# WeiZhang1988/YDORBSLAM

Measured on AMD Instinct MI355X. Metric: ORB extract+match Mkeypoints/sec, higher is better.
Workload: dtype u8

## Files before the change

### ydorbslam_amd/csrc/extract_kernels.hip.h

```cpp
#pragma once
#include <hip/hip_runtime.h>
#include <stdint.h>

#include "quadtree_core.h"
#include "quadtree_flat.h"

#pragma clang fp contract(off)

namespace ydorb {

constexpr int kPad = 19;
constexpr int kBorder = 16;
constexpr int kMaxLevels = 8;
constexpr int kTileMax = 72;
#ifndef QT_THREADS
#define QT_THREADS 512
#endif
constexpr int kQtThreads = QT_THREADS;

struct LevelDev {
  int w, h, pitch;
  int padOff;
  int blurOff, blurPitch;
  int cellBegin, nCells;
// ... 954 lines not shown
      const int i = t * NT + tid;
      if (i < n && kp[t] < nOut && mm[t] > 16) nodeBig[kp[t]] = 1;
    }
    static_assert(PER <= ITEMS, "the all-pairs candidates live in the first PER state registers");
#pragma unroll
    for (int t = 0; t < PER; t++) st[t] = (st[t] & 0xFFFF0000u) | (uint32_t)(kp[t] < nOut ? kp[t] : 0x7FFF);
    __syncthreads();
  }

#pragma unroll
  for (int g = 0; g < ITEMS / 4; g++) {
    if (!pairs && 4 * g * NT < n) {
      int key[4], slot[4];
#pragma unroll
      for (int jj = 0; jj < 4; jj++) { key[jj] = (int)(st[4 * g + jj] & 0xFFFu); slot[jj] = qf_off(Pn) + (key[jj] >> (2 * (D - Pn))); }
      for (int d = Pn - 1; d >= 1; d--) {
        const int off = qf_off(d), sh = 2 * (D - d);
#pragma unroll
        for (int jj = 0; jj < 4; jj++) {
          const int sl = off + (key[jj] >> sh);
          if (hist[sl] == 1) slot[jj] = sl;
        }
      }
#pragma unroll
      for (int jj = 0; jj < 4; jj++) st[4 * g + jj] = (st[4 * g + jj] & 0xFFFF0000u) | (uint32_t)slot[jj];
    }
  }
  if (!pairs) {
    const int TQ = ((1 << (2 * Pn)) - 1) / 3;
    const int per = (TQ + NT - 1) / NT;
    constexpr int MAXQ = ((1 << (2 * D)) - 1) / 3 / NT + 1;
    uint2 qv[MAXQ];
    int qslot[MAXQ];
    unsigned flags = 0, cntF = 0;
#pragma unroll
    for (int t = 0; t < MAXQ; t++) {
      qslot[t] = -1; qv[t] = make_uint2(0, 0);
      const int q = tid * per + t;
      if (t < per && q < TQ) {
        int d = Pn, start = 0;
        while (q >= start + (1 << (2 * (d - 1)))) { start += 1 << (2 * (d - 1)); d--; }
        const int pq = q - start;
        const int bq = pq ^ (int)(qt_flat_mask(d) >> 2);
        qslot[t] = qf_off(d) + 4 * bq;
        qv[t] = *reinterpret_cast<const QT_LDS uint2*>(hist + qslot[t]);
        const unsigned c[4] = {qv[t].x & 0xFFFFu, qv[t].x >> 16, qv[t].y & 0xFFFFu, qv[t].y >> 16};
        const unsigned sum = c[0] + c[1] + c[2] + c[3];
#pragma unroll
        for (int e = 0; e < 4; e++) {
          const unsigned cn = c[3 - e];
          const bool fl = sum >= 2 && (d == Pn ? cn >= 1 : cn == 1);
          flags |= (unsigned)fl << (4 * t + e);
          cntF += fl;
        }
      }
    }
    unsigned total;
    unsigned pos = block_scan_excl(cntF, &total);
    if ((int)total != K) { give_up(); return; }
#pragma unroll
    for (int t = 0; t < MAXQ; t++) {
      if (qslot[t] >= 0) {
        const unsigned c[4] = {qv[t].x & 0xFFFFu, qv[t].x >> 16, qv[t].y & 0xFFFFu, qv[t].y >> 16};
        unsigned o[4];
#pragma unroll
        for (int e = 0; e < 4; e++) {
          const unsigned cn = c[3 - e];
          unsigned v = 0x7FFFu;
          if ((flags >> (4 * t + e)) & 1u) {
            if ((int)pos < nOut) {
              v = pos | (cn > 16 ? 0x8000u : 0u);
              if (cn > 16) nodeBig[pos] = 1;
            }
            pos++;
          }
          o[3 - e] = v;
        }
        *reinterpret_cast<QT_LDS uint2*>(hist + qslot[t]) = make_uint2(o[0] | (o[1] << 16), o[2] | (o[3] << 16));
      }
    }
  }
  __syncthreads();

#pragma unroll
  for (int g = 0; g < ITEMS / 4; g++) {
    if (4 * g * NT < n) {
      unsigned pv[4];
#pragma unroll
      for (int jj = 0; jj < 4; jj++) pv[jj] = pairs ? st[4 * g + jj] & 0x7FFFu : hist[st[4 * g + jj] & 0xFFFFu] & 0x7FFFu;
#pragma unroll
      for (int jj = 0; jj < 4; jj++) {
        const int i = (4 * g + jj) * NT + tid;
        const bool ok = i < n && (int)pv[jj] < nOut;
        const unsigned k = ok ? pv[jj] : (unsigned)(quotaMax + 1);
        const uint32_t rs = st[4 * g + jj] & 0xFFFF0000u;
        __hip_atomic_fetch_max(nodeLo + k, ok ? rs | (0xFFFFu - (uint32_t)i) : 0u, __ATOMIC_RELAXED, __HIP_MEMORY_SCOPE_WORKGROUP);
        __hip_atomic_fetch_max(nodeHi + k, ok ? rs | (uint32_t)i : 0u, __ATOMIC_RELAXED, __HIP_MEMORY_SCOPE_WORKGROUP);
        st[4 * g + jj] = rs | (ok ? k : 0xFFFFu);
      }
    }
  }
  __syncthreads();
  for (int k = tid; k < nOut; k += NT) {
    const unsigned iLo = 0xFFFFu - (nodeLo[k] & 0xFFFFu), iHi = nodeHi[k] & 0xFFFFu;
    if (iLo == iHi || !nodeBig[k]) {
      outKp[k] = fetch((int)iLo);
    } else {
      const int s = atomicAdd(&sTieN, 1);
      if (s < kQfMaxTied) { sTieNode[s] = k; nodeBig[k] = (uint8_t)(2 + s); }
    }
  }
  __syncthreads();
  const int nTied = sTieN;
  if (nTied > kQfMaxTied) { give_up(); return; }
  if (nTied > 0) {
    const int slotCap = kQfTieCap / nTied;
    QT_LDS uint32_t* tKey = (QT_LDS uint32_t*)smem;
    QT_LDS uint32_t* tVal = tKey + kQfTieCap;
#pragma unroll
    for (int j = 0; j < ITEMS; j++) {
      if (j * NT < n) {
        const unsigned k = st[j] & 0xFFFFu;
        if (k != 0xFFFFu) {
          const unsigned tb = nodeBig[k];
          if (tb >= 2) {
            const int s = (int)tb - 2, idx = atomicAdd(&sTieCnt[s], 1);
            if (idx < slotCap) { tKey[s * slotCap + idx] = (uint32_t)(j * NT + tid); tVal[s * slotCap + idx] = st[j] >> 16; }
            else sFlag = 1;
          }
        }
      }
    }
    __syncthreads();
    if (sFlag) { give_up(); return; }
    for (int s = 0; s < nTied; s++) {
      const int m = sTieCnt[s];
      constexpr int MAXM = (kQfTieCap + NT - 1) / NT;
      int rk[MAXM];
      uint32_t oi[MAXM], rr[MAXM];
#pragma unroll
      for (int t = 0; t < MAXM; t++) {
        rk[t] = -1; oi[t] = 0; rr[t] = 0;
        const int e = tid + NT * t;
        if (e < m) {
          oi[t] = tKey[s * slotCap + e];
          rr[t] = tVal[s * slotCap + e];
          int r = 0;
          for (int u = 0; u < m; u++) r += tKey[s * slotCap + u] < oi[t];
          rk[t] = r;
        }
      }
      __syncthreads();
#pragma unroll
      for (int t = 0; t < MAXM; t++)
        if (rk[t] >= 0) { tKey[s * slotCap + rk[t]] = (rr[t] << 16) | (uint32_t)rk[t]; tVal[s * slotCap + rk[t]] = oi[t]; }
      __syncthreads();
    }
    if (tid < nTied) {
      const int m = sTieCnt[tid];
      const int best = qt_sort_front(tKey + tid * slotCap, m);
      outKp[sTieNode[tid]] = fetch((int)tVal[tid * slotCap + best]);
    }
  }
  if (tid == 0) { needPass[unit] = 0; lvlCount[unit] = nOut; }
}

__global__ __launch_bounds__(256) void k_blur(const uint8_t* __restrict__ pyr, size_t pyrFrameStride, uint8_t* __restrict__ blur,
                                              size_t blurFrameStride, PlanDev P) {
  constexpr int TW = kBlurTW, TH = kBlurTH, SH = TH + 6, SWW = 18;
  __shared__ uint32_t src[SH * SWW];
  __shared__ __align__(16) uint32_t hb[(SH / 2) * TW];
  int f = blockIdx.y, tileId = blockIdx.x;
  if ((f | 7) < (int)gridDim.y) {
    tileId = (f & 7) * (gridDim.x >> 3) + (blockIdx.x >> 3);
    f = (f & ~7) | (blockIdx.x & 7);
  }
  if (tileId >= P.blurTileBegin[P.nLevels]) return;
  int level = 0;
#pragma unroll
  for (int l = 1; l < kMaxLevels; l++)
    if (l < P.nLevels && tileId >= P.blurTileBegin[l]) level = l;
  tileId -= P.blurTileBegin[level];
  const LevelDev L = P.lv[level];
  const int tilesX = (L.w + TW - 1) / TW;
  const int ty = tileId / tilesX, tx = tileId - ty * tilesX;
  const int x0 = tx * TW, y0 = ty * TH;
  const uint8_t* padded = pyr + (size_t)f * pyrFrameStride + L.padOff;
  {
    const int r0 = threadIdx.x / SWW, wd = threadIdx.x - r0 * SWW;
    const int pcol = x0 + 16 + 4 * wd;
    const bool colOk = pcol < L.pitch;
    if (r0 < 14)
#pragma unroll
      for (int r = r0; r < SH; r += 14) {
        const int prow = min(y0 + r + kPad - 3, L.h + 2 * kPad - 1);
        src[r * SWW + wd] = colOk ? *reinterpret_cast<const uint32_t*>(padded + (size_t)prow * L.pitch + pcol) : 0u;
      }
  }
  __syncthreads();
  for (int task = threadIdx.x; task < (SH / 2) * (TW / 4); task += 256) {
    const int rp = task >> 4, g = task & 15;
    uint32_t o[2][4];
#pragma unroll
    for (int h = 0; h < 2; h++) {
      const int r = 2 * rp + h;
      const uint32_t w0 = src[r * SWW + g], w1 = src[r * SWW + g + 1], w2 = src[r * SWW + g + 2];
#pragma unroll
      for (int k = 0; k < 4; k++) {
        const uint32_t lo4 = k ? __builtin_amdgcn_alignbyte(w1, w0, k) : w0, hi4 = k ? __builtin_amdgcn_alignbyte(w2, w1, k) : w1;
        o[h][k] = __builtin_amdgcn_udot4(hi4, 0x00122230u, __builtin_amdgcn_udot4(lo4, 0x38302212u, 0u, false), false);
      }
    }
    *reinterpret_cast<uint4*>(&hb[rp * TW + g * 4]) =
        make_uint4(o[0][0] | (o[1][0] << 16), o[0][1] | (o[1][1] << 16), o[0][2] | (o[1][2] << 16), o[0][3] | (o[1][3] << 16));
  }
  __syncthreads();
  const int c4 = (threadIdx.x & 15) * 4;
#pragma unroll
  for (int r = threadIdx.x >> 4; r < TH; r += 16) {
    const int gy = y0 + r;
    if (!(gy < L.h && x0 + c4 < L.blurPitch)) continue;
    typedef unsigned short u16x2 __attribute__((ext_vector_type(2)));
    const bool odd = r & 1;
    const u16x2 k0 = odd ? u16x2{0, 18} : u16x2{18, 34}, k1 = odd ? u16x2{34, 48} : u16x2{48, 56};
    const u16x2 k2 = odd ? u16x2{56, 48} : u16x2{48, 34}, k3 = odd ? u16x2{34, 18} : u16x2{18, 0};
    const uint32_t* hp = &hb[(r >> 1) * TW + c4];
    const uint4 p0 = *reinterpret_cast<const uint4*>(hp), p1 = *reinterpret_cast<const uint4*>(hp + TW);
    const uint4 p2 = *reinterpret_cast<const uint4*>(hp + 2 * TW), p3 = *reinterpret_cast<const uint4*>(hp + 3 * TW);
    const uint32_t q0[4] = {p0.x, p0.y, p0.z, p0.w}, q1[4] = {p1.x, p1.y, p1.z, p1.w}, q2[4] = {p2.x, p2.y, p2.z, p2.w}, q3[4] = {p3.x, p3.y, p3.z, p3.w};
    uint32_t acc[4];
#pragma unroll
    for (int k = 0; k < 4; k++) {
      acc[k] = __builtin_amdgcn_udot2(__builtin_bit_cast(u16x2, q0[k]), k0, 32768u, false);
      acc[k] = __builtin_amdgcn_udot2(__builtin_bit_cast(u16x2, q1[k]), k1, acc[k], false);
      acc[k] = __builtin_amdgcn_udot2(__builtin_bit_cast(u16x2, q2[k]), k2, acc[k], false);
      acc[k] = __builtin_amdgcn_udot2(__builtin_bit_cast(u16x2, q3[k]), k3, acc[k], false);
    }
    const uint32_t out = (acc[0] >> 16) | ((acc[1] >> 16) << 8) | ((acc[2] >> 16) << 16) | ((acc[3] >> 16) << 24);
    *reinterpret_cast<uint32_t*>(blur + (size_t)f * blurFrameStride + L.blurOff + (size_t)gy * L.blurPitch + x0 + c4) = out;
  }
}

__device__ __forceinline__ float fast_atan2_deg(float y, float x) {
  const float p1 = 0.9997878412794807f * (float)(180 / 3.14159265358979323846);
  const float p3 = -0.3258083974640975f * (float)(180 / 3.14159265358979323846);
  const float p5 = 0.1555786518463281f * (float)(180 / 3.14159265358979323846);
  const float p7 = -0.04432655554792128f * (float)(180 / 3.14159265358979323846);
  const float eps = (float)2.2204460492503131e-16;
  const float ax = fabsf(x), ay = fabsf(y);
  float a, c, c2;
  if (ax >= ay) {
    c = __fdiv_rn(ay, __fadd_rn(ax, eps));
    c2 = __fmul_rn(c, c);
    a = __fmul_rn(__fadd_rn(__fmul_rn(__fadd_rn(__fmul_rn(__fadd_rn(__fmul_rn(p7, c2), p5), c2), p3), c2), p1), c);
  } else {
    c = __fdiv_rn(ax, __fadd_rn(ay, eps));
    c2 = __fmul_rn(c, c);
    a = __fsub_rn(90.f, __fmul_rn(__fadd_rn(__fmul_rn(__fadd_rn(__fmul_rn(__fadd_rn(__fmul_rn(p7, c2), p5), c2), p3), c2), p1), c));
  }
  if (x < 0) a = __fsub_rn(180.f, a);
  if (y < 0) a = __fsub_rn(360.f, a);
  return a;
}

__device__ __forceinline__ void sincos_det(float xf, float* sinOut, float* cosOut) {
  const double x = (double)xf;
  const double n = rint(__dmul_rn(x, 6.36619772367581382433e-01));
  const double r = __dsub_rn(__dsub_rn(x, __dmul_rn(n, 1.57079632673412561417e+00)), __dmul_rn(n, 6.07710050650619224932e-11));
  const double z = __dmul_rn(r, r);
  double p = __dmul_rn(z, 1.58969099521155010221e-10);
  p = __dadd_rn(p, -2.50507602534068634195e-08); p = __dmul_rn(p, z);
  p = __dadd_rn(p, 2.75573137070700676789e-06);  p = __dmul_rn(p, z);
  p = __dadd_rn(p, -1.98412698298579493134e-04); p = __dmul_rn(p, z);
  p = __dadd_rn(p, 8.33333333332248946124e-03);  p = __dmul_rn(p, z);
  p = __dadd_rn(p, -1.66666666666666324348e-01); p = __dmul_rn(p, z);
  p = __dmul_rn(p, r); p = __dadd_rn(p, r);
  double q = __dmul_rn(z, -1.13596475577881948265e-11);
  q = __dadd_rn(q, 2.08757232129817482790e-09);  q = __dmul_rn(q, z);
  q = __dadd_rn(q, -2.75573143513906633035e-07); q = __dmul_rn(q, z);
  q = __dadd_rn(q, 2.48015872894767294178e-05);  q = __dmul_rn(q, z);
  q = __dadd_rn(q, -1.38888888888741095749e-03); q = __dmul_rn(q, z);
  q = __dadd_rn(q, 4.16666666666666019037e-02);  q = __dmul_rn(q, z);
  q = __dmul_rn(q, z);
  double h = __dmul_rn(z, 0.5);
  h = __dsub_rn(h, q);
  h = __dsub_rn(1.0, h);
  const int quad = ((int)n) & 3;
  const double sv = quad == 0 ? p : quad == 1 ? h : quad == 2 ? -p : -h;
  const double cv = quad == 0 ? h : quad == 1 ? -p : quad == 2 ? -h : p;
  *sinOut = (float)sv;
  *cosOut = (float)cv;
}

__device__ __align__(16) const float kPatternDev[1024] = {
#include "orb_pattern_data.inc"
};

struct YdKeyPointDev { float x, y, size, angle, response; int octave, class_id; };

__global__ __launch_bounds__(256) void k_orient_describe(const uint8_t* __restrict__ pyr, size_t pyrFrameStride,
                                                         const uint8_t* __restrict__ blur, size_t blurFrameStride, PlanDev P,
                                                         const uint32_t* __restrict__ lvlKp, const int* __restrict__ lvlCount,
                                                         YdKeyPointDev* __restrict__ kps, uint8_t* __restrict__ desc, int cap,
                                                         int* __restrict__ nOut, float* __restrict__ lvlAngle) {
  const int lane = threadIdx.x & 63;
  int bx = blockIdx.x, f = blockIdx.y;
  if ((f | 7) < (int)gridDim.y) {
    bx = (f & 7) * (gridDim.x >> 3) + (blockIdx.x >> 3);
    f = (f & ~7) | (blockIdx.x & 7);
  }
  const int slot = bx * 4 + __builtin_amdgcn_readfirstlane(threadIdx.x >> 6);
  if (slot >= P.sumQuota) return;
  float4 pat[4];
#pragma unroll
  for (int t = 0; t < 4; t++) pat[t] = reinterpret_cast<const float4*>(kPatternDev)[t * 64 + lane];
  int level = 0;
#pragma unroll
  for (int l = 1; l < kMaxLevels; l++)
    if (l < P.nLevels && slot >= P.lv[l].kpOff) level = l;
  const uint32_t pk = __builtin_amdgcn_readfirstlane(lvlKp[(size_t)f * P.sumQuota + slot]);
  int before = 0, tot = 0, mine = 0;
#pragma unroll
  for (int l = 0; l < kMaxLevels; l++) {
    const int c = l < P.nLevels ? lvlCount[f * kMaxLevels + l] : 0;
    if (l < level) before += c;
    if (l == level) mine = c;
    tot += c;
  }
  if (slot == 0 && lane == 0) nOut[f] = min(tot, cap);
  const LevelDev L = P.lv[level];
  const int k = slot - L.kpOff;
  if (k >= mine) return;
  const int outIdx = before + k;
  if (outIdx >= cap) return;
  const int kx = qt_x(pk) + kBorder, ky = qt_y(pk) + kBorder;
  const uint8_t* roi = pyr + (size_t)f * pyrFrameStride + L.padOff + (size_t)kPad * L.pitch + kPad;
  const uint8_t* org = roi + (ptrdiff_t)(ky - 15) * L.pitch + (kx - 32);
  const int u = lane - 32;
  unsigned narrow = 0;
#pragma unroll
  for (int v = 1; v <= 15; v++) narrow |= (unsigned)(P.maxX[v] == 0) << v;
  int m10 = 0, m01 = 0;
  if (u >= -15 && u <= 15) m10 = u * org[(unsigned)(15 * L.pitch + lane)];
  if (lane >= 1 && lane <= 15 && ((narrow >> lane) & 1u)) {
    const int pos = org[(unsigned)((15 + lane) * L.pitch + 32)], neg = org[(unsigned)((15 - lane) * L.pitch + 32)];
    m01 = lane * (pos - neg);
  }
#pragma unroll
  for (int v = 1; v <= 15; v++) {
    const int d = P.maxX[v];
    if (d > 0 && u >= -d && u <= d) {
      const int pos = org[(unsigned)((15 + v) * L.pitch + lane)], neg = org[(unsigned)((15 - v) * L.pitch + lane)];
      m01 += v * (pos - neg);
      m10 += u * (pos + neg);
    }
  }
#pragma unroll
  for (int o = 32; o >= 1; o >>= 1) {
    m10 += __shfl_xor(m10, o, 64);
    m01 += __shfl_xor(m01, o, 64);
  }
  const float angle = fast_atan2_deg((float)m01, (float)m10);
  const float rad = __fmul_rn(angle, (float)(3.14159265358979323846 / 180.0));
  float sinB, cosA;
  sincos_det(rad, &sinB, &cosA);
  constexpr int kBias = 24;
  const uint8_t* bl = blur + (size_t)f * blurFrameStride + L.blurOff + (ptrdiff_t)(ky - kBias) * L.blurPitch + (kx - kBias);
  unsigned long long words[4];
#pragma unroll
  for (int t = 0; t < 4; t++) {
    const float4 pt = pat[t];
    const int r0 = __float2int_rn(__fadd_rn(__fmul_rn(pt.x, sinB), __fmul_rn(pt.y, cosA)));
    const int c0 = __float2int_rn(__fsub_rn(__fmul_rn(pt.x, cosA), __fmul_rn(pt.y, sinB)));
    const int r1 = __float2int_rn(__fadd_rn(__fmul_rn(pt.z, sinB), __fmul_rn(pt.w, cosA)));
    const int c1 = __float2int_rn(__fsub_rn(__fmul_rn(pt.z, cosA), __fmul_rn(pt.w, sinB)));
    const int t0 = bl[(unsigned)((r0 + kBias) * L.blurPitch + c0 + kBias)], t1 = bl[(unsigned)((r1 + kBias) * L.blurPitch + c1 + kBias)];
    words[t] = __ballot(t0 < t1);
  }
  if (lane < 4) {
    unsigned long long w = lane == 0 ? words[0] : lane == 1 ? words[1] : lane == 2 ? words[2] : words[3];
    reinterpret_cast<unsigned long long*>(desc + ((size_t)f * cap + outIdx) * 32)[lane] = w;
  }
  if (lane == 0) {
    YdKeyPointDev kp;
    kp.x = (float)kx;
    kp.y = (float)ky;
    if (level) { kp.x = __fmul_rn(kp.x, L.scale); kp.y = __fmul_rn(kp.y, L.scale); }
    kp.size = L.size;
    kp.angle = angle;
    kp.response = (float)qt_r(pk);
    kp.octave = level;
    kp.class_id = -1;
    kps[(size_t)f * cap + outIdx] = kp;
    lvlAngle[(size_t)f * P.sumQuota + slot] = angle;
  }
}


template <int KPW>
__global__ __launch_bounds__(256) void k_orient_describe_n(const uint8_t* __restrict__ pyr, size_t pyrFrameStride,
                                                           const uint8_t* __restrict__ blur, size_t blurFrameStride, PlanDev P,
                                                           const uint32_t* __restrict__ lvlKp, const int* __restrict__ lvlCount,
                                                           YdKeyPointDev* __restrict__ kps, uint8_t* __restrict__ desc, int cap,
                                                           int* __restrict__ nOut, float* __restrict__ lvlAngle) {
  const int lane = threadIdx.x & 63;
  int bx = blockIdx.x, f = blockIdx.y;
  if ((f | 7) < (int)gridDim.y) {
    bx = (f & 7) * (gridDim.x >> 3) + (blockIdx.x >> 3);
    f = (f & ~7) | (blockIdx.x & 7);
  }
  const int slot0 = (bx * 4 + __builtin_amdgcn_readfirstlane(threadIdx.x >> 6)) * KPW;
  if (slot0 >= P.sumQuota) return;
  float4 pat[4];
#pragma unroll
  for (int t = 0; t < 4; t++) pat[t] = reinterpret_cast<const float4*>(kPatternDev)[t * 64 + lane];
  int cnt[kMaxLevels], tot = 0;
#pragma unroll
  for (int l = 0; l < kMaxLevels; l++) { cnt[l] = l < P.nLevels ? lvlCount[f * kMaxLevels + l] : 0; tot += cnt[l]; }
  int level[KPW], outIdx[KPW];
  uint32_t pk[KPW];
  bool valid[KPW];
#pragma unroll
  for (int j = 0; j < KPW; j++) {
    const int slot = min(slot0 + j, P.sumQuota - 1);
    level[j] = 0;
#pragma unroll
    for (int l = 1; l < kMaxLevels; l++)
      if (l < P.nLevels && slot >= P.lv[l].kpOff) level[j] = l;
    pk[j] = __builtin_amdgcn_readfirstlane(lvlKp[(size_t)f * P.sumQuota + slot]);
  }
  if (slot0 == 0 && lane == 0) nOut[f] = min(tot, cap);
  bool any = false;
#pragma unroll
  for (int j = 0; j < KPW; j++) {
    int before = 0, mine = 0;
#pragma unroll
    for (int l = 0; l < kMaxLevels; l++) {
      if (l < level[j]) before += cnt[l];
      if (l == level[j]) mine = cnt[l];
    }
    const int k = slot0 + j - P.lv[level[j]].kpOff;
    outIdx[j] = before + k;
    valid[j] = slot0 + j < P.sumQuota && k < mine && outIdx[j] < cap;
    any = any || valid[j];
  }
  if (!any) return;
  int firstValid = 0;
#pragma unroll
  for (int j = KPW - 1; j >= 0; j--) if (valid[j]) firstValid = j;
#pragma unroll
  for (int j = 0; j < KPW; j++)
    if (!valid[j]) {
#pragma unroll
      for (int i = 0; i < KPW; i++) if (i == firstValid) { pk[j] = pk[i]; level[j] = level[i]; }
    }
  int kx[KPW], ky[KPW], pitch[KPW];
  const uint8_t* org[KPW];
#pragma unroll
  for (int j = 0; j < KPW; j++) {
    const LevelDev& L = P.lv[level[j]];
    kx[j] = qt_x(pk[j]) + kBorder; ky[j] = qt_y(pk[j]) + kBorder;
    pitch[j] = L.pitch;
    const uint8_t* roi = pyr + (size_t)f * pyrFrameStride + L.padOff + (size_t)kPad * L.pitch + kPad;
    org[j] = roi + (ptrdiff_t)(ky[j] - 15) * L.pitch + (kx[j] - 32);
  }
  const int u = lane - 32;
  unsigned narrow = 0;
#pragma unroll
  for (int v = 1; v <= 15; v++) narrow |= (unsigned)(P.maxX[v] == 0) << v;
  int m10[KPW], m01[KPW];
#pragma unroll
  for (int j = 0; j < KPW; j++) {
    m10[j] = 0; m01[j] = 0;
    if (u >= -15 && u <= 15) m10[j] = u * org[j][(unsigned)(15 * pitch[j] + lane)];
    if (lane >= 1 && lane <= 15 && ((narrow >> lane) & 1u)) {
      const int pos = org[j][(unsigned)((15 + lane) * pitch[j] + 32)], neg = org[j][(unsigned)((15 - lane) * pitch[j] + 32)];
      m01[j] = lane * (pos - neg);
    }
  }
#pragma unroll
  for (int v = 1; v <= 15; v++) {
    const int d = P.maxX[v];
    if (d > 0 && u >= -d && u <= d) {
#pragma unroll
      for (int j = 0; j < KPW; j++) {
        const int pos = org[j][(unsigned)((15 + v) * pitch[j] + lane)], neg = org[j][(unsigned)((15 - v) * pitch[j] + lane)];
        m01[j] += v * (pos - neg);
        m10[j] += u * (pos + neg);
      }
    }
  }
#pragma unroll
  for (int o = 32; o >= 1; o >>= 1) {
#pragma unroll
    for (int j = 0; j < KPW; j++) {
      m10[j] += __shfl_xor(m10[j], o, 64);
      m01[j] += __shfl_xor(m01[j], o, 64);
    }
  }
  constexpr int kBias = 24;
  float angle[KPW];
  int tA[KPW][4], tB[KPW][4];
#pragma unroll
  for (int j = 0; j < KPW; j++) {
    const LevelDev& L = P.lv[level[j]];
    angle[j] = fast_atan2_deg((float)m01[j], (float)m10[j]);
    const float rad = __fmul_rn(angle[j], (float)(3.14159265358979323846 / 180.0));
    float sinB, cosA;
    sincos_det(rad, &sinB, &cosA);
    const uint8_t* bl = blur + (size_t)f * blurFrameStride + L.blurOff + (ptrdiff_t)(ky[j] - kBias) * L.blurPitch + (kx[j] - kBias);
#pragma unroll
    for (int t = 0; t < 4; t++) {
      const float4 pt = pat[t];
      const int r0 = __float2int_rn(__fadd_rn(__fmul_rn(pt.x, sinB), __fmul_rn(pt.y, cosA)));
      const int c0 = __float2int_rn(__fsub_rn(__fmul_rn(pt.x, cosA), __fmul_rn(pt.y, sinB)));
      const int r1 = __float2int_rn(__fadd_rn(__fmul_rn(pt.z, sinB), __fmul_rn(pt.w, cosA)));
      const int c1 = __float2int_rn(__fsub_rn(__fmul_rn(pt.z, cosA), __fmul_rn(pt.w, sinB)));
      tA[j][t] = bl[(unsigned)((r0 + kBias) * L.blurPitch + c0 + kBias)];
      tB[j][t] = bl[(unsigned)((r1 + kBias) * L.blurPitch + c1 + kBias)];
    }
  }
#pragma unroll
  for (int j = 0; j < KPW; j++) {
    unsigned long long words[4];
#pragma unroll
    for (int t = 0; t < 4; t++) words[t] = __ballot(tA[j][t] < tB[j][t]);
    if (!valid[j]) continue;
    const LevelDev& L = P.lv[level[j]];
    if (lane < 4) {
      unsigned long long w = lane == 0 ? words[0] : lane == 1 ? words[1] : lane == 2 ? words[2] : words[3];
      reinterpret_cast<unsigned long long*>(desc + ((size_t)f * cap + outIdx[j]) * 32)[lane] = w;
    }
    if (lane == 0) {
      YdKeyPointDev kp;
      kp.x = (float)kx[j];
      kp.y = (float)ky[j];
      if (level[j]) { kp.x = __fmul_rn(kp.x, L.scale); kp.y = __fmul_rn(kp.y, L.scale); }
      kp.size = L.size;
      kp.angle = angle[j];
      kp.response = (float)qt_r(pk[j]);
      kp.octave = level[j];
      kp.class_id = -1;
      kps[(size_t)f * cap + outIdx[j]] = kp;
      lvlAngle[(size_t)f * P.sumQuota + slot0 + j] = angle[j];
    }
  }
}

}
```

### ydorbslam_amd/csrc/orb_extractor.hip

```cpp
#include <hip/hip_runtime.h>
#include <cstdlib>

#include <algorithm>
#include <cmath>
#include <cstdarg>
#include <cstdio>
#include <cstring>
#include <string>
#include <vector>

#include "../../include/ydorb/c_api.h"
#include "extract_kernels.hip.h"
#include "host_buffers.h"
#include "ydorb_host.h"

using namespace ydorb;

namespace {

inline int cvRoundF(float v) { return (int)lrintf(v); }
inline int cvFloorF(float v) { int i = (int)v; return i - (i > v); }
inline int alignUp(int v, int a) { return (v + a - 1) / a * a; }
inline size_t alignUpZ(size_t v, size_t a) { return (v + a - 1) / a * a; }

struct HostPlan {
  int w = 0, h = 0;
  PlanDev dev{};
  std::vector<CellDev> cells;
  size_t pyrFrameStride = 0, blurFrameStride = 0, qtFrameStride = 0;
  int maxCellDim = 0;
  int levelCellDim[kMaxLevels]{};
  struct QtLevel { int nodeCap, candCap; size_t lds; int items; bool passOk; } qt[kMaxLevels]{};
  size_t qtLdsMax = 0;
  size_t qtPassLds = 0;
  int qtPassNodes = 0;
  std::vector<int> tabInt;
  std::vector<short> tabShort;
  struct TabOff { int xofs, yofs, alpha, beta; } tab[kMaxLevels]{};
  struct FusedLevel { bool on = false; int shift = 0, padOff = 0, colOff = 0, rowOff = 0; } fused[kMaxLevels];
  std::vector<PyrPadEntry> padTab;
  std::vector<PyrColEntry> colTab;
  std::vector<int2> rowTab;
};

enum Stage { ST_PYR = 0, ST_FAST, ST_QT, ST_BLUR, ST_DESC, ST_COUNT };
const char* kStageNames[ST_COUNT] = {"pyramid", "fast_cells", "blur", "quadtree_after_blur", "orient_describe"};

struct TablePtrs { CellDev* cells; int* tabInt; short* tabShort; PyrPadEntry* padTab; PyrColEntry* colTab; int2* rowTab; };
size_t layTables(const HostPlan& P, void* base, TablePtrs& t) {
  Carve a(base);
  a.take(t.cells, P.cells.size()); a.take(t.tabInt, P.tabInt.size()); a.take(t.tabShort, P.tabShort.size());
  a.take(t.padTab, P.padTab.size()); a.take(t.colTab, P.colTab.size()); a.take(t.rowTab, P.rowTab.size());
  return a.L.bytes;
}

struct WorkPtrs {
  uint8_t *pyr, *blur; uint32_t *cellCount, *cellCand, *qtCand; uint16_t* qtNode; uint8_t* nodeScratch; uint32_t* lvlKp; float* lvlAngle; int* lvlCount;
  uint8_t* needPass; int *lvlMaxN, *status, *passList;
};
size_t layWork(const HostPlan& P, size_t B, void* base, WorkPtrs& w) {
  const PlanDev& D = P.dev;
  Carve a(base);
  a.take(w.pyr, P.pyrFrameStride * B); a.take(w.blur, P.blurFrameStride * B);
  a.take(w.cellCount, D.nCellsTotal * B); a.take(w.cellCand, (size_t)D.nCellsTotal * D.cellCap * B);
  a.take(w.qtCand, 2 * P.qtFrameStride * B); a.take(w.qtNode, 2 * P.qtFrameStride * B); a.take(w.nodeScratch, D.nodeTabFrameStride * B);
  a.take(w.lvlKp, D.sumQuota * B); a.take(w.lvlAngle, D.sumQuota * B); a.take(w.lvlCount, kMaxLevels * B);
  a.take(w.needPass, kMaxLevels * B); a.take(w.lvlMaxN, kMaxLevels + 1); a.take(w.status, 1); a.take(w.passList, kMaxLevels * B + 1);
  return a.L.bytes;
}

struct IoPtrs { uint8_t* img; YdKeyPoint* kps; uint8_t* desc; int* nOut; };
size_t layIo(size_t imgBytes, size_t Q, size_t B, void* base, IoPtrs& p) {
  static_assert(sizeof(YdKeyPoint) == sizeof(YdKeyPointDev), "one layout for the device and the pinned staging");
  Carve a(base);
  a.take(p.img, imgBytes * B); a.take(p.kps, Q * B); a.take(p.desc, 32 * Q * B); a.take(p.nOut, B);
  return a.L.bytes;
}

}

struct ydorb_extractor {
  YdExtractorConfig cfg{};
  std::vector<float> sf, isf, sf2, isf2;
  std::vector<int> perLevel;
  int maxX[16]{};
  int sumQuota = 0;
  hipStream_t stream = nullptr;
  hipStream_t qtStream[kMaxLevels]{};
  hipEvent_t evFork = nullptr, evJoin[kMaxLevels]{};
  hipEvent_t evFast[kMaxLevels]{};
  int descKpw = 2;
  bool qtInline = false;
  int fastGroups = 1;
  HostPlan plan;
  bool planValid = false;
  int batchCap = 0;
  size_t imgBytes = 0;
  Mem tables;
  Mem work;
  Mem io; PinnedMem hIo;
  PinnedMem hSync;
  PinnedMem h_pyr;
  TablePtrs tab{};
  WorkPtrs d{};
  IoPtrs dIo{}, hIoAt{};
  int *h_lvlMaxN = nullptr, *h_status = nullptr;
  std::vector<Mem*> buffers() { return {&tables, &work, &io, &hIo, &hSync, &h_pyr}; }
  hipStream_t lastStream = nullptr;
  int lastFrames = 0;
  bool noFusedPads = false;
  bool profiling = false;
  bool profPending = false;
  bool forcePassQuadtree = false;
  hipEvent_t ev[ST_COUNT + 1]{};
  double stageMs[ST_COUNT]{};
  int stageCalls = 0;
};

namespace {

void release(ydorb_extractor* e) {
  for (Mem* b : e->buffers()) b->release();
  e->planValid = false;
  e->lastStream = nullptr; e->lastFrames = 0;
}

int syncStreams(ydorb_extractor* e) {
  HIPCHK(hipStreamSynchronize(e->stream));
  if (e->lastStream && e->lastStream != e->stream) HIPCHK(hipStreamSynchronize(e->lastStream));
  return YDORB_OK;
}


static int qfItemsFor(long want) { return want <= 8L * kQfThreads ? 8 : want <= 16L * kQfThreads ? 16 : 32; }

void buildFusedLevel(HostPlan& P, int l) {
  const PlanDev& D = P.dev;
  const LevelDev& L = D.lv[l];
  HostPlan::FusedLevel& F = P.fused[l];
  F.on = false;
  if (L.w < 20 || L.h < 20) return;
  const int nd = (L.w + 2 * kPad + 3) >> 2;
  auto srcOf = [&](int p) { return p < kPad ? 2 * kPad - p : p < kPad + L.w ? -1 : p < L.w + 2 * kPad ? 2 * L.w + 2 * kPad - 2 - p : -2; };
  int shift = -1;
  for (int sft = 0; sft < 64 && shift < 0; sft++) {
    bool ok = true;
    for (int c = 0; c < nd && ok; c++)
      for (int j = 0; j < 4; j++) {
        const int sp = srcOf(4 * c + j);
        if (sp >= 0 && ((sp >> 2) + sft) >> 6 != (c + sft) >> 6) ok = false;
      }
    if (ok) shift = sft;
  }
  if (shift < 0) return;
  std::vector<PyrColEntry> col;
  if (l > 0) {
    const LevelDev& Lp = D.lv[l - 1];
    const int* xofs = P.tabInt.data() + P.tab[l].xofs;
    const short* alpha = P.tabShort.data() + P.tab[l].alpha;
    col.resize(nd);
    for (int c = 0; c < nd; c++) {
      const int dx0 = std::min(std::max(4 * c - kPad, 0), L.w - 1);
      for (int b = 0; b < 4; b++) {
        const int dx = std::min(std::max(4 * c - kPad + b, 0), L.w - 1);
        const int off = xofs[dx] - xofs[dx0];
        if (off < 0 || off > 6 || xofs[dx0] + 7 >= Lp.w + kPad) return;
        col[c].sel[b] = (uint32_t)off | 0x0c000c00u | ((uint32_t)(off + 1) << 16);
        col[c].ab[b] = (uint32_t)(uint16_t)alpha[2 * dx] | ((uint32_t)(uint16_t)alpha[2 * dx + 1] << 16);
      }
    }
  }
  F.shift = shift;
  F.padOff = (int)P.padTab.size();
  for (int c = 0; c < nd; c++) {
    int dA = -1, dB = -1;
    for (int j = 0; j < 4; j++) {
      const int sp = srcOf(4 * c + j);
      if (sp < 0) continue;
      const int d = sp >> 2;
      if (dA < 0 || d == dA) dA = d;
      else dB = d;
    }
    PyrPadEntry pe{};
    pe.laneA4 = 4u * (unsigned)(((dA < 0 ? c : dA) + shift) & 63);
    pe.laneB4 = 4u * (unsigned)(((dB < 0 ? c : dB) + shift) & 63);
    pe.selM = 0; pe.selF = 0;
    for (int j = 0; j < 4; j++) {
      const int sp = srcOf(4 * c + j);
      uint32_t m = 0x0c, f;
      if (sp == -1) f = (uint32_t)j;
      else if (sp == -2) f = 0x0c;
      else { m = (uint32_t)(sp & 3) + ((sp >> 2) == dA ? 4u : 0u); f = 4u + (uint32_t)j; }
      pe.selM |= m << (8 * j);
      pe.selF |= f << (8 * j);
    }
    P.padTab.push_back(pe);
  }
  if (l > 0) {
    F.colOff = (int)P.colTab.size();
    P.colTab.insert(P.colTab.end(), col.begin(), col.end());
    F.rowOff = (int)P.rowTab.size();
    const int* yofs = P.tabInt.data() + P.tab[l].yofs;
    const short* beta = P.tabShort.data() + P.tab[l].beta;
    const int rows = alignUp(L.h, 4 * kPyrRowsF);
    for (int y = 0; y < rows; y++) {
      const int dy = std::min(y, L.h - 1);
      P.rowTab.push_back(make_int2(yofs[dy], (int)((uint32_t)(uint16_t)beta[2 * dy] | ((uint32_t)(uint16_t)beta[2 * dy + 1] << 16))));
    }
  }
  F.on = true;
}

int buildPlan(ydorb_extractor* e, int w, int h, HostPlan& P) {
  P = HostPlan();
  P.w = w; P.h = h;
  PlanDev& D = P.dev;
  D.nLevels = e->cfg.n_levels;
  for (int v = 0; v < 16; v++) D.maxX[v] = e->maxX[v];
  size_t padOff = 0, blurOff = 0;
  int kpOff = 0, candOff = 0, maxCellDim = 0;
  for (int l = 0; l < D.nLevels; l++) {
    LevelDev& L = D.lv[l];
    L.w = cvRoundF((float)w * e->isf[l]);
    L.h = cvRoundF((float)h * e->isf[l]);
    if (L.w < 1 || L.h < 1 || L.w > 4000 || L.h > 4000) {
      set_error("level %d size %dx%d out of the supported range (1..4000)", l, L.w, L.h);
      return YDORB_ERR_UNSUPPORTED;
    }
    L.pitch = alignUp(L.w + 2 * kPad, 64);
    L.padOff = (int)padOff;
    padOff += alignUpZ((size_t)(L.h + 2 * kPad) * L.pitch, 256);
    L.blurPitch = alignUp(L.w, 64);
    L.blurOff = (int)blurOff;
    blurOff += alignUpZ((size_t)L.h * L.blurPitch, 256);
    L.quota = e->perLevel[l];
    L.kpOff = kpOff;
    kpOff += L.quota;
    L.scale = e->sf[l];
    L.size = (float)(int)(31 * e->sf[l]);
    L.cellBegin = (int)P.cells.size();
    const int minB = kBorder, maxBX = L.w - kBorder, maxBY = L.h - kBorder;
    const float width = (float)(maxBX - minB), height = (float)(maxBY - minB);
    const int colsNum = (int)(width / 30.0f), rowsNum = (int)(height / 30.0f);
    if (colsNum > 0 && rowsNum > 0) {
      const int cellW = (int)ceilf(width / colsNum), cellH = (int)ceilf(height / rowsNum);
      maxCellDim = std::max(maxCellDim, std::max(cellW, cellH));
      P.levelCellDim[l] = std::max(cellW, cellH);
      for (int i = 0; i < rowsNum; i++) {
        const float iniY = (float)(minB + i * cellH);
        float maxY = iniY + cellH + 6;
        if (iniY >= maxBY - 3) continue;
        if (maxY > maxBY) maxY = (float)maxBY;
        for (int j = 0; j < colsNum; j++) {
          const float iniX = (float)(minB + j * cellW);
          float maxX = iniX + cellW + 6;
          if (iniX >= maxBX - 6) continue;
          if (maxX > maxBX) maxX = (float)maxBX;
          CellDev c{};
          c.level = (short)l;
          c.x0 = (short)iniX; c.y0 = (short)iniY; c.x1 = (short)maxX; c.y1 = (short)maxY;
          c.srcOff = L.padOff + (kPad + c.y0) * L.pitch + kPad + c.x0;
          P.cells.push_back(c);
        }
      }
    }
    L.nCells = (int)P.cells.size() - L.cellBegin;
    if (l > 0) {
      const LevelDev& Lp = D.lv[l - 1];
      const double scale_x = 1. / ((double)L.w / Lp.w), scale_y = 1. / ((double)L.h / Lp.h);
      P.tab[l].xofs = (int)P.tabInt.size();
      P.tab[l].alpha = (int)P.tabShort.size();
      for (int dx = 0; dx < L.w; dx++) {
        float fx = (float)((dx + 0.5) * scale_x - 0.5);
        int sx = cvFloorF(fx);
        fx -= sx;
        if (sx < 0) { fx = 0; sx = 0; }
        if (sx >= Lp.w - 1) { fx = 0; sx = Lp.w - 1; }
        P.tabInt.push_back(sx);
        P.tabShort.push_back((short)cvRoundF((1.f - fx) * 2048));
        P.tabShort.push_back((short)cvRoundF(fx * 2048));
      }
      P.tab[l].yofs = (int)P.tabInt.size();
      P.tab[l].beta = (int)P.tabShort.size();
      for (int dy = 0; dy < L.h; dy++) {
        float fy = (float)((dy + 0.5) * scale_y - 0.5);
        int sy = cvFloorF(fy);
        fy -= sy;
        P.tabInt.push_back(sy);
        P.tabShort.push_back((short)cvRoundF((1.f - fy) * 2048));
        P.tabShort.push_back((short)cvRoundF(fy * 2048));
      }
    }
  }
  if (maxCellDim + 6 > kTileMax) {
    set_error("cell size %d exceeds the FAST tile (%d)", maxCellDim, kTileMax - 6);
    return YDORB_ERR_UNSUPPORTED;
  }
  D.nCellsTotal = (int)P.cells.size();
  P.maxCellDim = maxCellDim;
  D.cellCap = alignUp(std::max(((maxCellDim + 1) / 2) * ((maxCellDim + 1) / 2), 64), 64);
  D.sumQuota = kpOff;
  for (int l = 0; l < D.nLevels; l++) {
    D.lv[l].candOff = candOff;
    candOff += D.lv[l].nCells * D.cellCap;
  }
  for (int l = 0; l < D.nLevels && !e->noFusedPads; l++) buildFusedLevel(P, l);
  D.borderBegin[0] = 0;
  for (int l = 0; l < kMaxLevels; l++)
    D.borderBegin[l + 1] = D.borderBegin[l] + (l < D.nLevels && !P.fused[l].on ? alignUp(2 * kPad * (D.lv[l].pitch / 4) + 12 * D.lv[l].h, 256) : 0);
  D.blurTileBegin[0] = 0;
  for (int l = 0; l < kMaxLevels; l++)
    D.blurTileBegin[l + 1] = D.blurTileBegin[l] + (l < D.nLevels ? ((D.lv[l].w + kBlurTW - 1) / kBlurTW) * ((D.lv[l].h + kBlurTH - 1) / kBlurTH) : 0);
  P.pyrFrameStride = padOff;
  P.blurFrameStride = blurOff;
  P.qtFrameStride = (size_t)candOff;
  for (int l = 0; l < D.nLevels; l++) {
    const LevelDev& L = D.lv[l];
    HostPlan::QtLevel& Q = P.qt[l];
    Q.nodeCap = 4 * std::max(L.quota, 1);
    const long band = (long)std::max(L.w - 2 * kBorder, 1) * std::max(L.h - 2 * kBorder, 1);
    Q.candCap = (int)std::min<long>(4608, std::max<long>(512, band / 22)) / 64 * 64;
    Q.lds = (size_t)Q.nodeCap * 48 + (size_t)Q.candCap * 12 + (size_t)(L.nCells + 1) * 4;
    if (Q.lds > 150 * 1024) {
      Q.candCap = 0;
      Q.lds = (size_t)Q.nodeCap * 48 + (size_t)(L.nCells + 1) * 4;
    }
    Q.passOk = Q.lds <= 150 * 1024;
    if (Q.passOk) {
      P.qtLdsMax = std::max(P.qtLdsMax, Q.lds);
      P.qtPassLds = std::max(P.qtPassLds, (size_t)Q.nodeCap * 48 + (size_t)(L.nCells + 1) * 4);
      P.qtPassNodes = std::max(P.qtPassNodes, Q.nodeCap);
      D.lv[l].nodeTabOff = -1;
    } else {
      if (Q.nodeCap > 65535) { set_error("n_features=%d: level %d would need %d quad-tree nodes (max 65535)", e->cfg.n_features, l, Q.nodeCap); return YDORB_ERR_UNSUPPORTED; }
      D.lv[l].nodeTabOff = (int)D.nodeTabFrameStride;
      D.nodeTabFrameStride += (unsigned)alignUpZ((size_t)Q.nodeCap * 48, 256);
      Q.candCap = 0;
      Q.lds = (size_t)(L.nCells + 1) * 4 + 64;
      P.qtLdsMax = std::max(P.qtLdsMax, Q.lds);
      P.qtPassLds = std::max(P.qtPassLds, Q.lds);
    }
    Q.items = qfItemsFor((long)((double)band / (45.0 - 3.5 * l)) + 64);
  }
  P.qtPassLds = std::max<size_t>(P.qtPassLds, 1024);
  return YDORB_OK;
}

size_t fastGeom(const HostPlan& P, int la, int lb, FastLds& fl, bool& narrow) {
  int dim = 1;
  for (int l = la; l < lb; l++) dim = std::max(dim, P.levelCellDim[l]);
  const int maxT = dim + 6, maxB = dim;
  narrow = maxT <= 44;
  const int pitch = narrow ? 48 : 80;
  fl.tileBytes = alignUp((maxT + 3) * pitch, 16);
  fl.scoreBytes = alignUp((maxB + 2) * (maxB + 2) + 4, 16);
  fl.listBytes = alignUp(2 * maxB * maxB, 16);
  return (size_t)4 * (fl.tileBytes + fl.scoreBytes + fl.listBytes);
}

template <class T> void copyTable(T* dst, const std::vector<T>& v) { if (!v.empty()) memcpy(dst, v.data(), sizeof(T) * v.size()); }

int ensurePlan(ydorb_extractor* e, int w, int h, int nFrames) {
  if (e->planValid && e->plan.w == w && e->plan.h == h && nFrames <= e->batchCap) return YDORB_OK;
  int rc = syncStreams(e);
  if (rc) return rc;
  HostPlan P;
  if ((rc = buildPlan(e, w, h, P))) return rc;
  release(e);
  const size_t B = std::max(nFrames, std::max(1, e->cfg.max_batch));
  const PlanDev& D = P.dev;
  std::vector<uint8_t> hTables(layTables(P, nullptr, e->tab));
  if ((rc = e->tables.alloc(hTables.size())) || (rc = e->work.alloc(layWork(P, B, nullptr, e->d))) ||
      (rc = e->hSync.alloc(sizeof(int) * (kMaxLevels + 2)))) return rc;
  layWork(P, B, e->work.p, e->d);
  e->h_lvlMaxN = e->hSync.as<int>();
  e->h_status = e->h_lvlMaxN + kMaxLevels + 1;
  memset(e->hSync.p, 0, e->hSync.cap);
  TablePtrs ht;
  layTables(P, hTables.data(), ht);
  copyTable(ht.cells, P.cells); copyTable(ht.tabInt, P.tabInt); copyTable(ht.tabShort, P.tabShort);
  copyTable(ht.padTab, P.padTab); copyTable(ht.colTab, P.colTab); copyTable(ht.rowTab, P.rowTab);
  layTables(P, e->tables.p, e->tab);
  if (!hTables.empty()) HIPCHK(hipMemcpyAsync(e->tables.p, hTables.data(), hTables.size(), hipMemcpyHostToDevice, e->stream));
  HIPCHK(hipMemsetAsync(e->d.pyr, 0, P.pyrFrameStride * B, e->stream));
  HIPCHK(hipMemsetAsync(e->d.needPass, 0, (uint8_t*)(e->d.passList + 1) - e->d.needPass, e->stream));
  HIPCHK(hipStreamSynchronize(e->stream));
  e->plan = P;
  e->batchCap = (int)B;
  e->imgBytes = (size_t)w * h;
  {
    FastLds fl; bool narrow;
    const size_t dynAll = fastGeom(P, 0, D.nLevels, fl, narrow);
    if (dynAll > 48 * 1024) {
      HIPCHK(hipFuncSetAttribute(reinterpret_cast<const void*>(k_fast_cells<48>), hipFuncAttributeMaxDynamicSharedMemorySize, (int)dynAll));
      HIPCHK(hipFuncSetAttribute(reinterpret_cast<const void*>(k_fast_cells<80>), hipFuncAttributeMaxDynamicSharedMemorySize, (int)dynAll));
    }
  }
  if (std::max(P.qtLdsMax, P.qtPassLds) > 48 * 1024)
  {
    HIPCHK(hipFuncSetAttribute(reinterpret_cast<const void*>(k_quadtree), hipFuncAttributeMaxDynamicSharedMemorySize, (int)std::max(P.qtLdsMax, P.qtPassLds)));
    HIPCHK(hipFuncSetAttribute(reinterpret_cast<const void*>(k_quadtree_list), hipFuncAttributeMaxDynamicSharedMemorySize, (int)std::max(P.qtLdsMax, P.qtPassLds)));
  }
  {
    int qmax = 1, tabLen = 2;
    for (int l = 0; l < D.nLevels; l++) { qmax = std::max(qmax, D.lv[l].quota); tabLen = std::max(tabLen, std::max(D.lv[l].w - 2 * kBorder, 0) + std::max(D.lv[l].h - 2 * kBorder, 0) + 2); }
    const size_t ldsFast = std::min<size_t>(qt_fast_lds_bytes(qmax, tabLen), 150 * 1024);
    if (ldsFast > 48 * 1024) {
      HIPCHK(hipFuncSetAttribute(reinterpret_cast<const void*>(k_qt_fast<8>), hipFuncAttributeMaxDynamicSharedMemorySize, (int)ldsFast));
      HIPCHK(hipFuncSetAttribute(reinterpret_cast<const void*>(k_qt_fast<16>), hipFuncAttributeMaxDynamicSharedMemorySize, (int)ldsFast));
      HIPCHK(hipFuncSetAttribute(reinterpret_cast<const void*>(k_qt_fast<32>), hipFuncAttributeMaxDynamicSharedMemorySize, (int)ldsFast));
    }
  }
  e->planValid = true;
  return YDORB_OK;
}

int ensureIo(ydorb_extractor* e) {
  if (e->io.p && e->hIo.p) return YDORB_OK;
  const size_t bytes = layIo(e->imgBytes, e->sumQuota, e->batchCap, nullptr, e->dIo);
  int rc;
  if ((rc = e->io.alloc(bytes)) || (rc = e->hIo.alloc(bytes))) return rc;
  layIo(e->imgBytes, e->sumQuota, e->batchCap, e->io.p, e->dIo);
  layIo(e->imgBytes, e->sumQuota, e->batchCap, e->hIo.p, e->hIoAt);
  return YDORB_OK;
}

void collectProfile(ydorb_extractor* e);

static void retuneQuadtree(ydorb_extractor* e) {
  HostPlan& P = e->plan;
  for (int l = 0; l < P.dev.nLevels; l++) {
    const int seen = e->h_lvlMaxN[l];
    if (seen > 0) P.qt[l].items = qfItemsFor((long)seen + seen / 8 + 32);
  }
}

int enqueue(ydorb_extractor* e, const uint8_t* d_img, int stride, size_t frameStride, int nFrames, YdKeyPointDev* d_kps,
            uint8_t* d_desc, int cap, int* d_nOut, hipStream_t s) {
  retuneQuadtree(e);
  const HostPlan& P = e->plan;
  const PlanDev& D = P.dev;
  const bool prof = e->profiling;
  if (prof) {
    if (e->profPending && hipEventQuery(e->ev[ST_COUNT]) == hipSuccess) collectProfile(e);
    e->profPending = false;
    HIPCHK(hipEventRecord(e->ev[0], s));
  }
  {
    const LevelDev& L0 = D.lv[0];
    auto fusedGrid = [&](const LevelDev& L, int shift) {
      return dim3((((L.w + 2 * kPad + 3) >> 2) + shift + 63) / 64, (L.h + 4 * kPyrRowsF - 1) / (4 * kPyrRowsF), nFrames);
    };
    if (P.fused[0].on) {
      hipLaunchKernelGGL(k_pyr_level0_f, fusedGrid(L0, P.fused[0].shift), dim3(256), 0, s, d_img, stride, frameStride, e->d.pyr, P.pyrFrameStride, L0,
                         e->tab.padTab + P.fused[0].padOff, P.fused[0].shift);
    } else {
      dim3 g((L0.pitch / 4 + 63) / 64, (L0.h + 4 * kPyrRows - 1) / (4 * kPyrRows), nFrames);
      hipLaunchKernelGGL(k_pyr_level0, g, dim3(256), 0, s, d_img, stride, frameStride, e->d.pyr, P.pyrFrameStride, L0);
    }
    for (int l = 1; l < D.nLevels; l++) {
      const LevelDev& L = D.lv[l];
      const double scaleX = 1. / ((double)L.w / D.lv[l - 1].w);
      if (P.fused[l].on) {
        const HostPlan::FusedLevel& F = P.fused[l];
        hipLaunchKernelGGL(k_pyr_resize_f, fusedGrid(L, F.shift), dim3(256), 0, s, e->d.pyr, P.pyrFrameStride, D.lv[l - 1], L, scaleX,
                           e->tab.colTab + F.colOff, e->tab.padTab + F.padOff, e->tab.rowTab + F.rowOff, F.shift);
      } else {
        dim3 gl((L.pitch / 4 + 63) / 64, (L.h + 4 * kPyrRows - 1) / (4 * kPyrRows), nFrames);
        hipLaunchKernelGGL(k_pyr_resize, gl, dim3(256), 0, s, e->d.pyr, P.pyrFrameStride, D.lv[l - 1], L, scaleX,
                           e->tab.tabShort + P.tab[l].alpha, e->tab.tabInt + P.tab[l].yofs, e->tab.tabShort + P.tab[l].beta);
      }
    }
    if (D.borderBegin[D.nLevels] > 0)
      hipLaunchKernelGGL(k_pyr_borders, dim3(D.borderBegin[D.nLevels] / 256, nFrames), dim3(256), 0, s, e->d.pyr, P.pyrFrameStride, D);
  }
  if (prof) HIPCHK(hipEventRecord(e->ev[1], s));
  hipEvent_t fastEv[kMaxLevels]{};
  int grpFirst[kMaxLevels]{}, grpEnd[kMaxLevels]{}, nGroups = 0;
  {
    const int thr = std::min(std::max(e->cfg.ini_fast_thr, 0), 255);
    int l0 = 0;
    for (int g = 0; g < e->fastGroups && l0 < D.nLevels; g++) {
      const int l1 = g == e->fastGroups - 1 ? D.nLevels : l0 + 1;
      const int c0 = D.lv[l0].cellBegin, c1 = D.lv[l1 - 1].cellBegin + D.lv[l1 - 1].nCells;
      if (c1 > c0 && D.nCellsTotal > 0) {
        FastLds fl; bool narrow;
        const size_t dyn = fastGeom(P, l0, l1, fl, narrow);
        const dim3 grid(((c1 - c0 + 3) / 4 + 7) / 8 * 8, nFrames);
        if (narrow) hipLaunchKernelGGL(k_fast_cells<48>, grid, dim3(256), dyn, s, e->d.pyr, P.pyrFrameStride, D, e->tab.cells, c0, c1, thr, fl, e->d.cellCount, e->d.cellCand);
        else hipLaunchKernelGGL(k_fast_cells<80>, grid, dim3(256), dyn, s, e->d.pyr, P.pyrFrameStride, D, e->tab.cells, c0, c1, thr, fl, e->d.cellCount, e->d.cellCand);
      }
      HIPCHK(hipEventRecord(e->evFast[l0], s));
      fastEv[l0] = e->evFast[l0];
      grpFirst[nGroups] = l0; grpEnd[nGroups] = l1; nGroups++;
      for (int l = l0 + 1; l < l1; l++) fastEv[l] = e->evFast[l0];
      l0 = l1;
    }
  }
  if (prof) HIPCHK(hipEventRecord(e->ev[2], s));
  HIPCHK(hipEventRecord(e->evFork, s));
  hipLaunchKernelGGL(k_blur, dim3((D.blurTileBegin[D.nLevels] + 7) / 8 * 8, nFrames), dim3(256), 0, s, e->d.pyr, P.pyrFrameStride, e->d.blur,
                     P.blurFrameStride, D);
  if (prof) HIPCHK(hipEventRecord(e->ev[3], s));
  bool anyFast = false;
  for (int g = 0; g < nGroups; g++) {
    const int l0 = grpFirst[g], l1 = grpEnd[g];
    const hipStream_t qs = e->qtInline ? s : e->qtStream[g % kMaxLevels];
    if (!e->qtInline) HIPCHK(hipStreamWaitEvent(qs, fastEv[l0] ? fastEv[l0] : e->evFork, 0));
    int items = 8, qmax = 1, tabLen = 2;
    for (int l = l0; l < l1; l++) {
      items = std::max(items, P.qt[l].items); qmax = std::max(qmax, D.lv[l].quota);
      tabLen = std::max(tabLen, std::max(D.lv[l].w - 2 * kBorder, 0) + std::max(D.lv[l].h - 2 * kBorder, 0) + 2);
    }
    const size_t lds = qt_fast_lds_bytes(qmax, tabLen);
    if (!e->forcePassQuadtree && lds <= 150 * 1024) {
      const dim3 grid(nFrames, l1 - l0);
#define YD_QT_FAST(IT) hipLaunchKernelGGL(k_qt_fast<IT>, grid, dim3(kQfThreads), lds, qs, D, e->d.cellCount, e->d.cellCand, l0, qmax, tabLen, e->d.lvlKp, \
                                          e->d.lvlCount, e->d.needPass, e->d.lvlMaxN, e->d.passList, e->d.passList + 1)
      if (items <= 8) YD_QT_FAST(8);
      else if (items <= 16) YD_QT_FAST(16);
      else YD_QT_FAST(32);
#undef YD_QT_FAST
      anyFast = true;
    } else {
      for (int l = l0; l < l1; l++) {
        const HostPlan::QtLevel& Q = P.qt[l];
        hipLaunchKernelGGL(k_quadtree, dim3(1, nFrames), dim3(kQtThreads), Q.lds, qs, D, e->d.cellCount, e->d.cellCand, e->d.qtCand, e->d.qtNode,
                           P.qtFrameStride, Q.nodeCap, Q.candCap, l, e->d.lvlKp, e->d.lvlCount, e->d.status, e->d.nodeScratch);
      }
    }
    if (!e->qtInline) HIPCHK(hipEventRecord(e->evJoin[g], qs));
  }
  if (!e->qtInline) for (int g = 0; g < nGroups; g++) HIPCHK(hipStreamWaitEvent(s, e->evJoin[g], 0));
  if (anyFast) {
    const int seen = e->h_lvlMaxN[kMaxLevels];
    const int listGrid = std::max(1, std::min({kQtPassWorkgroups, D.nLevels * nFrames, seen + seen / 4}));
    hipLaunchKernelGGL(k_quadtree_list, dim3(listGrid), dim3(kQtListThreads), P.qtPassLds, s, D, e->d.cellCount, e->d.cellCand,
                       e->d.qtCand, e->d.qtNode, P.qtFrameStride, -std::max(P.qtPassNodes, 1), e->d.lvlKp, e->d.lvlCount, e->d.status, e->d.passList,
                       e->d.passList + 1, e->d.nodeScratch, e->d.lvlMaxN + kMaxLevels);
    HIPCHK(hipMemsetAsync(e->d.passList, 0, sizeof(int), s));
  }
  if (prof) HIPCHK(hipEventRecord(e->ev[4], s));
  {
    const int kpw = e->descKpw;
    const dim3 gd(((D.sumQuota + 4 * kpw - 1) / (4 * kpw) + 7) / 8 * 8, nFrames);
#define YD_DESC(K) hipLaunchKernelGGL((k_orient_describe_n<K>), gd, dim3(256), 0, s, e->d.pyr, P.pyrFrameStride, e->d.blur, P.blurFrameStride, D, \
                                         e->d.lvlKp, e->d.lvlCount, d_kps, d_desc, cap, d_nOut, e->d.lvlAngle)
    if (kpw == 1)
      hipLaunchKernelGGL(k_orient_describe, gd, dim3(256), 0, s, e->d.pyr, P.pyrFrameStride, e->d.blur,
                         P.blurFrameStride, D, e->d.lvlKp, e->d.lvlCount, d_kps, d_desc, cap, d_nOut, e->d.lvlAngle);
    else if (kpw == 2) YD_DESC(2);
    else YD_DESC(4);
#undef YD_DESC
  }
  if (prof) { HIPCHK(hipEventRecord(e->ev[5], s)); e->profPending = true; }
  HIPCHK(hipMemcpyAsync(e->h_lvlMaxN, e->d.lvlMaxN, sizeof(int) * (kMaxLevels + 1), hipMemcpyDeviceToHost, s));
  HIPCHK(hipGetLastError());
  e->lastFrames = nFrames;
  e->lastStream = s;
  return YDORB_OK;
}

int checkStatus(ydorb_extractor* e) {
  if (*e->h_status == 1) { set_error("more than 65535 FAST candidates in one pyramid level"); return YDORB_ERR_CAPACITY; }
  if (*e->h_status == 3) { set_error("a pyramid level needs the pass quad-tree kernel (more candidates than LDS slots, or a very deep tree) but its quota is too large for that kernel's LDS node table"); return YDORB_ERR_CAPACITY; }
  if (*e->h_status) { set_error("quad-tree node table overflow (status %d)", *e->h_status); return YDORB_ERR_CAPACITY; }
  return YDORB_OK;
}

void collectProfile(ydorb_extractor* e) {
  if (!e->profiling || !e->profPending) return;
  e->profPending = false;
  for (int i = 0; i < ST_COUNT; i++) {
    float ms = 0;
    if (hipEventElapsedTime(&ms, e->ev[i], e->ev[i + 1]) == hipSuccess) e->stageMs[i] += ms;
  }
  e->stageCalls++;
}

}

int ydorb::extractor_pyramid_view(const ydorb_extractor* e, PyramidView* v) {
  if (!e || !v || !e->planValid || e->lastFrames < 1) { set_error("the extractor holds no pyramid (no call yet)"); return YDORB_ERR_INVALID_ARG; }
  v->device = e->cfg.device; v->nLevels = e->cfg.n_levels; v->frames = e->lastFrames; v->frameStride = (long long)e->plan.pyrFrameStride;
  v->stream = e->stream;
  for (int l = 0; l < e->cfg.n_levels; l++) {
    const LevelDev& L = e->plan.dev.lv[l];
    v->roi[l] = e->d.pyr + L.padOff + (size_t)kPad * L.pitch + kPad;
    v->w[l] = L.w; v->h[l] = L.h; v->pitch[l] = L.pitch;
    v->scale[l] = e->sf[l]; v->invScale[l] = e->isf[l];
    v->quota[l] = e->perLevel[l];
  }
  return YDORB_OK;
}

extern "C" {

int ydorb_extractor_create(const YdExtractorConfig* cfg, ydorb_extractor_t** out) {
  if (!cfg || !out) { set_error("null argument"); return YDORB_ERR_INVALID_ARG; }
  *out = nullptr;
  if (cfg->n_levels < 1 || cfg->n_levels > kMaxLevels || cfg->n_features < 1 || !(cfg->scale_factor > 1.0f)) {
    set_error("unsupported extractor config (n_levels 1..8, n_features >= 1, scale_factor > 1)");
    return YDORB_ERR_INVALID_ARG;
  }
  int rc = ydorb::require_device(cfg->device);
  if (rc) return rc;
  ydorb_extractor* e = new ydorb_extractor();
  e->cfg = *cfg;
  if (const char* v = getenv("YDORB_QT_PASS")) e->forcePassQuadtree = v[0] == '1';
  if (const char* v = getenv("YDORB_PYR_FUSED")) e->noFusedPads = v[0] == '0';
  e->descKpw = cfg->max_batch <= 8 ? 1 : 4;
  if (const char* v = getenv("YDORB_DESC_KPW")) e->descKpw = atoi(v) == 1 ? 1 : atoi(v) == 4 ? 4 : 2;
  e->cfg.min_fast_thr = cfg->ini_fast_thr;
  const int L = cfg->n_levels;
  const float s = cfg->scale_factor;
  int per = (int)round(cfg->n_features * (1 - 1.0 / s) / (1.0 - pow(1.0 / s, L)));
  int sum = 0;
  for (int i = 0; i < L; i++) {
    e->sf.push_back((float)pow(s, i));
    e->sf2.push_back((float)pow(s, 2 * i));
    e->isf.push_back((float)pow(s, -i));
    e->isf2.push_back((float)pow(s, -2 * i));
    if (i < L - 1) {
      e->perLevel.push_back(per);
      sum += per;
      per = (int)round((float)per / s);
    } else {
      e->perLevel.push_back(std::max(cfg->n_features - sum, 0));
    }
  }
  e->sumQuota = 0;
  for (int q : e->perLevel) e->sumQuota += q;
  {
    const int half = 15;
    std::vector<int> mx(half + 1, 0);
    const int maxY = (int)floor(half * sqrt(2.0) / 2.0 + 1.0), minY = (int)ceil(half * sqrt(2.0) / 2.0);
    for (int v = 0; v <= maxY; v++) mx.push_back((int)round(sqrt((double)half * half + (double)v * v)));
    for (int v = half, i = 0; v >= minY; v--) {
      while (mx[i] == mx[i + 1]) i++;
      mx[v] = i;
      i++;
    }
    for (int v = 0; v < 16; v++) e->maxX[v] = mx[v];
  }
  if (hipStreamCreateWithFlags(&e->stream, hipStreamNonBlocking) != hipSuccess) {
    set_error("hipStreamCreate failed");
    delete e;
    return YDORB_ERR_HIP;
  }
  for (auto& ev : e->ev) (void)hipEventCreate(&ev);
  (void)hipEventCreateWithFlags(&e->evFork, hipEventDisableTiming);
  for (int l = 0; l < kMaxLevels; l++) {
    const char* qtEnv = getenv("YDORB_QT_STREAMS");
    e->qtInline = (qtEnv && atoi(qtEnv) == 0) || (cfg->flags & YDORB_EXTRACTOR_SINGLE_STREAM);
    const int nQt = std::max(1, std::min(qtEnv ? atoi(qtEnv) : (cfg->max_batch <= 8 ? (int)kMaxLevels : 2), (int)kMaxLevels));
    if (l < nQt) (void)hipStreamCreateWithFlags(&e->qtStream[l], hipStreamNonBlocking);
    else e->qtStream[l] = e->qtStream[l % nQt];
    (void)hipEventCreateWithFlags(&e->evJoin[l], hipEventDisableTiming);
    (void)hipEventCreateWithFlags(&e->evFast[l], hipEventDisableTiming);
  }
  {
    const char* g = getenv("YDORB_FAST_GROUPS");
    e->fastGroups = std::max(1, std::min(g ? atoi(g) : (cfg->max_batch <= 8 ? 1 : 2), (int)kMaxLevels));
  }
  *out = e;
  return YDORB_OK;
}

void ydorb_extractor_destroy(ydorb_extractor_t* e) {
  if (!e) return;
  (void)hipSetDevice(e->cfg.device);
  if (e->stream) (void)hipStreamSynchronize(e->stream);
  release(e);
  for (auto& ev : e->ev) if (ev) (void)hipEventDestroy(ev);
  for (int l = 0; l < kMaxLevels; l++) {
    if (e->qtStream[l]) {
      bool shared = false;
      for (int k = 0; k < l; k++) shared = shared || e->qtStream[k] == e->qtStream[l];
      if (!shared) { (void)hipStreamSynchronize(e->qtStream[l]); (void)hipStreamDestroy(e->qtStream[l]); }
    }
    if (e->evJoin[l]) (void)hipEventDestroy(e->evJoin[l]);
    if (e->evFast[l]) (void)hipEventDestroy(e->evFast[l]);
  }
  if (e->evFork) (void)hipEventDestroy(e->evFork);
  if (e->stream) (void)hipStreamDestroy(e->stream);
  delete e;
}

int ydorb_extractor_tables(const ydorb_extractor_t* e, float* scale, float* inv_scale, float* scale_sq, float* inv_scale_sq,
                           int32_t* per_level) {
  if (!e) { set_error("null handle"); return YDORB_ERR_INVALID_ARG; }
  for (int i = 0; i < e->cfg.n_levels; i++) {
    if (scale) scale[i] = e->sf[i];
    if (inv_scale) inv_scale[i] = e->isf[i];
    if (scale_sq) scale_sq[i] = e->sf2[i];
    if (inv_scale_sq) inv_scale_sq[i] = e->isf2[i];
    if (per_level) per_level[i] = e->perLevel[i];
  }
  return YDORB_OK;
}

int ydorb_extractor_max_keypoints(const ydorb_extractor_t* e) { return e ? e->sumQuota : YDORB_ERR_INVALID_ARG; }

int ydorb_extract_batch_device(ydorb_extractor_t* e, const uint8_t* d_img, int32_t w, int32_t h, int32_t stride, size_t frame_stride,
                               int32_t n_frames, YdKeyPoint* d_kps, uint8_t* d_desc, int32_t cap, int32_t* d_n_out, void* stream) {
  if (!e || !d_img || !d_kps || !d_desc || !d_n_out || w <= 0 || h <= 0 || n_frames <= 0 || stride < w) {
    set_error("invalid argument");
    return YDORB_ERR_INVALID_ARG;
  }
  if (cap < e->sumQuota) { set_error("cap %d < max keypoints %d", cap, e->sumQuota); return YDORB_ERR_CAPACITY; }
  HIPCHK(hipSetDevice(e->cfg.device));
  int rc = ensurePlan(e, w, h, n_frames);
  if (rc) return rc;
  return enqueue(e, d_img, stride, frame_stride, n_frames, reinterpret_cast<YdKeyPointDev*>(d_kps), d_desc, cap, d_n_out,
                 stream ? (hipStream_t)stream : e->stream);
}

int ydorb_extractor_synchronize(ydorb_extractor_t* e) {
  if (!e) { set_error("null handle"); return YDORB_ERR_INVALID_ARG; }
  HIPCHK(hipSetDevice(e->cfg.device));
  int rc = syncStreams(e);
  if (rc || !e->planValid) return rc;
  HIPCHK(hipMemcpy(e->h_status, e->d.status, sizeof(int), hipMemcpyDeviceToHost));
  rc = checkStatus(e);
  if (rc) HIPCHK(hipMemset(e->d.status, 0, sizeof(int)));
  return rc;
}

int ydorb_extract_batch(ydorb_extractor_t* e, const uint8_t* img, int32_t w, int32_t h, int32_t stride, size_t frame_stride,
                        int32_t n_frames, YdKeyPoint* kps, uint8_t* desc, int32_t cap, int32_t* n_out) {
  if (!e || !n_out) { set_error("null argument"); return YDORB_ERR_INVALID_ARG; }
  if (!img || w <= 0 || h <= 0 || n_frames <= 0) {
    for (int f = 0; f < std::max(n_frames, 0); f++) n_out[f] = 0;
    return YDORB_OK;
  }
  if (!kps || !desc || stride < w) { set_error("invalid argument"); return YDORB_ERR_INVALID_ARG; }
  HIPCHK(hipSetDevice(e->cfg.device));
  int rc = ensurePlan(e, w, h, n_frames);
  if (rc || (rc = ensureIo(e))) return rc;
  const int Q = e->sumQuota;
  YdKeyPointDev* d_kps = reinterpret_cast<YdKeyPointDev*>(e->dIo.kps);
  for (int f = 0; f < n_frames; f++)
    for (int y = 0; y < h; y++) memcpy(e->hIoAt.img + (size_t)f * e->imgBytes + (size_t)y * w, img + f * frame_stride + (size_t)y * stride, w);
  HIPCHK(hipMemcpyAsync(e->dIo.img, e->hIoAt.img, e->imgBytes * n_frames, hipMemcpyHostToDevice, e->stream));
  rc = enqueue(e, e->dIo.img, w, e->imgBytes, n_frames, d_kps, e->dIo.desc, Q, e->dIo.nOut, e->stream);
  if (rc) return rc;
  HIPCHK(hipMemcpyAsync(e->hIoAt.nOut, e->dIo.nOut, sizeof(int) * n_frames, hipMemcpyDeviceToHost, e->stream));
  HIPCHK(hipMemcpyAsync(e->h_status, e->d.status, sizeof(int), hipMemcpyDeviceToHost, e->stream));
  HIPCHK(hipMemcpyAsync(e->hIoAt.kps, d_kps, sizeof(YdKeyPoint) * (size_t)Q * n_frames, hipMemcpyDeviceToHost, e->stream));
  HIPCHK(hipMemcpyAsync(e->hIoAt.desc, e->dIo.desc, (size_t)32 * Q * n_frames, hipMemcpyDeviceToHost, e->stream));
  HIPCHK(hipStreamSynchronize(e->stream));
  collectProfile(e);
  rc = checkStatus(e);
  if (rc) {
    HIPCHK(hipMemset(e->d.status, 0, sizeof(int)));
    return rc;
  }
  for (int f = 0; f < n_frames; f++) {
    const int n = e->hIoAt.nOut[f];
    if (n > cap) { set_error("frame %d has %d keypoints, caller capacity %d", f, n, cap); return YDORB_ERR_CAPACITY; }
    memcpy(kps + (size_t)f * cap, e->hIoAt.kps + (size_t)f * Q, sizeof(YdKeyPoint) * n);
    memcpy(desc + (size_t)f * cap * 32, e->hIoAt.desc + (size_t)f * Q * 32, (size_t)32 * n);
    n_out[f] = n;
  }
  return YDORB_OK;
}

int ydorb_extract(ydorb_extractor_t* e, const uint8_t* img, int32_t w, int32_t h, int32_t stride, YdKeyPoint* kps, uint8_t* desc,
                  int32_t cap, int32_t* n_out) {
  return ydorb_extract_batch(e, img, w, h, stride, 0, 1, kps, desc, cap, n_out);
}

int ydorb_extractor_pyramid(const ydorb_extractor_t* e, int32_t frame, int32_t level, const uint8_t** d_roi, int32_t* w, int32_t* h,
                            int32_t* stride) {
  if (!e || !e->planValid || frame < 0 || frame >= e->lastFrames || level < 0 || level >= e->cfg.n_levels) {
    set_error("no pyramid for frame %d level %d", frame, level);
    return YDORB_ERR_INVALID_ARG;
  }
  const LevelDev& L = e->plan.dev.lv[level];
  if (d_roi) *d_roi = e->d.pyr + (size_t)frame * e->plan.pyrFrameStride + L.padOff + (size_t)kPad * L.pitch + kPad;
  if (w) *w = L.w;
  if (h) *h = L.h;
  if (stride) *stride = L.pitch;
  return YDORB_OK;
}

int ydorb_extractor_read_level(ydorb_extractor_t* e, int32_t frame, int32_t level, uint8_t* dst, size_t dst_bytes) {
  const uint8_t* roi;
  int w, h, stride;
  int rc = ydorb_extractor_pyramid(e, frame, level, &roi, &w, &h, &stride);
  if (rc) return rc;
  const size_t need = (size_t)(w + 2 * kPad) * (h + 2 * kPad);
  if (!dst || dst_bytes < need) { set_error("need %zu bytes", need); return YDORB_ERR_CAPACITY; }
  HIPCHK(hipSetDevice(e->cfg.device));
  HIPCHK(hipStreamSynchronize(e->stream));
  HIPCHK(hipMemcpy2D(dst, w + 2 * kPad, roi - (size_t)kPad * stride - kPad, stride, w + 2 * kPad, h + 2 * kPad, hipMemcpyDeviceToHost));
  return YDORB_OK;
}

int ydorb_extractor_read_pyramid(ydorb_extractor_t* e, int32_t frame, uint8_t* const* dst_levels, const size_t* dst_bytes, int32_t n_levels) {
  if (!e || !e->planValid || frame < 0 || frame >= e->lastFrames || !dst_levels || !dst_bytes || n_levels < 1 || n_levels > e->cfg.n_levels) {
    set_error("invalid argument");
    return YDORB_ERR_INVALID_ARG;
  }
  const HostPlan& P = e->plan;
  for (int l = 0; l < n_levels; l++) {
    const LevelDev& L = P.dev.lv[l];
    const size_t need = (size_t)(L.w + 2 * kPad) * (L.h + 2 * kPad);
    if (!dst_levels[l] || dst_bytes[l] < need) { set_error("level %d needs %zu bytes", l, need); return YDORB_ERR_CAPACITY; }
  }
  HIPCHK(hipSetDevice(e->cfg.device));
  if (const int rc = e->h_pyr.ensure(P.pyrFrameStride)) return rc;
  const uint8_t* h_pyr = e->h_pyr.as<uint8_t>();
  hipStream_t s = e->lastStream ? e->lastStream : e->stream;
  HIPCHK(hipMemcpyAsync(e->h_pyr.p, e->d.pyr + (size_t)frame * P.pyrFrameStride, P.pyrFrameStride, hipMemcpyDeviceToHost, s));
  HIPCHK(hipStreamSynchronize(s));
  for (int l = 0; l < n_levels; l++) {
    const LevelDev& L = P.dev.lv[l];
    const int rowBytes = L.w + 2 * kPad;
    for (int y = 0; y < L.h + 2 * kPad; y++) memcpy(dst_levels[l] + (size_t)y * rowBytes, h_pyr + L.padOff + (size_t)y * L.pitch, rowBytes);
  }
  return YDORB_OK;
}

int ydorb_extractor_debug_read(ydorb_extractor_t* e, int32_t what, int32_t frame, int32_t level, void* dst, size_t dst_bytes,
                               size_t* written) {
  if (!e || !e->planValid || frame < 0 || frame >= e->lastFrames || level < 0 || level >= e->cfg.n_levels || !dst || !written) {
    set_error("invalid argument");
    return YDORB_ERR_INVALID_ARG;
  }
  HIPCHK(hipSetDevice(e->cfg.device));
  HIPCHK(hipStreamSynchronize(e->stream));
  const HostPlan& P = e->plan;
  const PlanDev& D = P.dev;
  const LevelDev& L = D.lv[level];
  if (what == 0) {
    const size_t need = (size_t)L.w * L.h;
    if (dst_bytes < need) { set_error("need %zu bytes", need); return YDORB_ERR_CAPACITY; }
    HIPCHK(hipMemcpy2D(dst, L.w, e->d.blur + (size_t)frame * P.blurFrameStride + L.blurOff, L.blurPitch, L.w, L.h, hipMemcpyDeviceToHost));
    *written = need;
    return YDORB_OK;
  }
  if (what == 1) {
    std::vector<uint32_t> cnt(L.nCells), buf((size_t)L.nCells * D.cellCap);
    if (L.nCells) {
      HIPCHK(hipMemcpy(cnt.data(), e->d.cellCount + (size_t)frame * D.nCellsTotal + L.cellBegin, sizeof(uint32_t) * L.nCells, hipMemcpyDeviceToHost));
      HIPCHK(hipMemcpy(buf.data(), e->d.cellCand + ((size_t)frame * D.nCellsTotal + L.cellBegin) * D.cellCap,
                       sizeof(uint32_t) * buf.size(), hipMemcpyDeviceToHost));
    }
    YdKeyPoint* o = (YdKeyPoint*)dst;
    size_t n = 0;
    for (int c = 0; c < L.nCells; c++)
      for (uint32_t i = 0; i < cnt[c]; i++) {
        if ((n + 1) * sizeof(YdKeyPoint) > dst_bytes) { set_error("candidate buffer too small"); return YDORB_ERR_CAPACITY; }
        const uint32_t pk = buf[(size_t)c * D.cellCap + i];
        o[n++] = YdKeyPoint{(float)qt_x(pk), (float)qt_y(pk), 7.f, -1.f, (float)qt_r(pk), 0, -1};
      }
    *written = n * sizeof(YdKeyPoint);
    return YDORB_OK;
  }
  if (what == 2) {
    int counts[kMaxLevels];
    HIPCHK(hipMemcpy(counts, e->d.lvlCount + frame * kMaxLevels, sizeof(counts), hipMemcpyDeviceToHost));
    const int n = counts[level];
    if ((size_t)n * sizeof(YdKeyPoint) > dst_bytes) { set_error("keypoint buffer too small"); return YDORB_ERR_CAPACITY; }
    std::vector<uint32_t> pk(std::max(n, 1));
    std::vector<float> ang(std::max(n, 1));
    if (n) {
      HIPCHK(hipMemcpy(pk.data(), e->d.lvlKp + (size_t)frame * D.sumQuota + L.kpOff, sizeof(uint32_t) * n, hipMemcpyDeviceToHost));
      HIPCHK(hipMemcpy(ang.data(), e->d.lvlAngle + (size_t)frame * D.sumQuota + L.kpOff, sizeof(float) * n, hipMemcpyDeviceToHost));
    }
    YdKeyPoint* o = (YdKeyPoint*)dst;
    for (int i = 0; i < n; i++)
      o[i] = YdKeyPoint{(float)(qt_x(pk[i]) + kBorder), (float)(qt_y(pk[i]) + kBorder), L.size, ang[i], (float)qt_r(pk[i]), level, -1};
    *written = (size_t)n * sizeof(YdKeyPoint);
    return YDORB_OK;
  }
  if (what == 3) {
    if (dst_bytes < 1) { set_error("need 1 byte"); return YDORB_ERR_CAPACITY; }
    uint8_t v = 1;
    int qmaxAll = 1, tabAll = 2;
    for (int l = 0; l < D.nLevels; l++) { qmaxAll = std::max(qmaxAll, D.lv[l].quota); tabAll = std::max(tabAll, std::max(D.lv[l].w - 2 * kBorder, 0) + std::max(D.lv[l].h - 2 * kBorder, 0) + 2); }
    if (!e->forcePassQuadtree && qt_fast_lds_bytes(qmaxAll, tabAll) <= 150 * 1024)
      HIPCHK(hipMemcpy(&v, e->d.needPass + (size_t)frame * kMaxLevels + level, 1, hipMemcpyDeviceToHost));
    *(uint8_t*)dst = v;
    *written = 1;
    return YDORB_OK;
  }
  set_error("unknown debug stage %d", what);
  return YDORB_ERR_INVALID_ARG;
}

int ydorb_extractor_set_profiling(ydorb_extractor_t* e, int32_t on) {
  if (!e) return YDORB_ERR_INVALID_ARG;
  e->profiling = on != 0;
  for (double& m : e->stageMs) m = 0;
  e->stageCalls = 0;
  return YDORB_OK;
}

int ydorb_extractor_stage_times(ydorb_extractor_t* e, int32_t max_stages, const char** names, float* ms, int32_t* n_stages) {
  if (!e || !n_stages) return YDORB_ERR_INVALID_ARG;
  if (e->profiling && e->profPending) {
    if (hipEventSynchronize(e->ev[ST_COUNT]) == hipSuccess) collectProfile(e);
  }
  const int n = std::min<int>(max_stages, ST_COUNT);
  for (int i = 0; i < n; i++) {
    if (names) names[i] = kStageNames[i];
    if (ms) ms[i] = e->stageCalls ? (float)(e->stageMs[i] / e->stageCalls) : 0.f;
  }
  *n_stages = n;
  return YDORB_OK;
}

}
```

### ydorbslam_amd/csrc/orb_matcher.hip

```cpp
#include <hip/hip_runtime.h>

#include <algorithm>
#include <cstdlib>
#include <cmath>
#include <cstring>
#include <vector>

#include "../../include/ydorb/c_api.h"
#include "frustum_kernels.hip.h"
#include "host_buffers.h"
#include "match_kernels.hip.h"
#include "stereo_kernels.hip.h"
#include "ydorb_host.h"

using namespace ydorb;

namespace {

int launchGridBuild(int nFrames, int cap, hipStream_t s, const FrameDev* frames) {
  const size_t dyn = sizeof(int16_t) * (size_t)std::max(cap, 0);
  if (dyn > 48 * 1024)
    HIPCHK(hipFuncSetAttribute(reinterpret_cast<const void*>(k_grid_build), hipFuncAttributeMaxDynamicSharedMemorySize, (int)dyn));
  hipLaunchKernelGGL(k_grid_build, dim3(nFrames), dim3(256), dyn, s, frames, cap);
  HIPCHK(hipGetLastError());
  return YDORB_OK;
}

__global__ void k_hamming_rows(const uint8_t* a, const uint8_t* b, int n, int* out) {
  const int i = blockIdx.x * 256 + threadIdx.x;
  if (i < n) out[i] = hamming256(a + (size_t)i * 32, b + (size_t)i * 32);
}

enum { MS_GRID = 0, MS_GATHER, MS_RESOLVE, MS_COUNT };
const char* kMatchStageNames[MS_COUNT] = {"grid_build", "gather_distances", "resolve"};

constexpr size_t kTakenPad = 31;

template <class Lay> int layOut(Mem& arena, Lay lay) {
  const int rc = arena.ensure(lay(nullptr));
  if (rc == YDORB_OK) lay(arena.p);
  return rc;
}

struct BatchPtrs {
  FrameDev* frames; CallDev* calls; float *sf, *ident;
  QueryDev* queries; uint8_t* taken; int* matchQ; int2* qInfo; uint2* qPre; unsigned* heads;
  int *cellStart, *cellIdx; float4* sortedKp; uint8_t* sortedDesc;
  uint32_t* pool;
};
size_t layBatch(size_t cap, size_t nCalls, size_t nFrames, size_t poolPerCall, void* base, BatchPtrs& p) {
  Carve a(base);
  a.take(p.frames, nFrames); a.take(p.calls, nCalls); a.take(p.sf, 8); a.take(p.ident, 6 * nCalls);
  a.take(p.queries, cap * nCalls); a.take(p.taken, cap * nCalls + kTakenPad); a.take(p.matchQ, cap * nCalls); a.take(p.qInfo, cap * nCalls);
  a.take(p.qPre, cap * nCalls); a.take(p.heads, nCalls); a.take(p.cellStart, (kGridCells + 1) * nFrames); a.take(p.cellIdx, cap * nFrames);
  a.take(p.sortedKp, cap * nFrames); a.take(p.sortedDesc, 32 * cap * nFrames);
  a.take(p.pool, poolPerCall * nCalls);
  return a.L.bytes;
}

struct ProjPtrs {
  int* status; FrameDev* frame; CallDev* call;
  KeyPointDev* kps; uint8_t* desc; float* rightX; int *cellStart, *cellIdx; float4* sortedKp; uint8_t* sortedDesc;
  QueryDev* queries; uint8_t *qdesc, *taken; int *assigned, *matchQ; int2* qInfo; uint2* qPre;
  uint8_t *table, *track;
};
size_t layProjection(size_t n, bool stereo, size_t nq, size_t tableBytes, size_t trackBytes, void* base, ProjPtrs& p) {
  Carve a(base);
  a.take(p.status, 16); a.take(p.frame, 1); a.take(p.call, 1);
  a.take(p.kps, n); a.take(p.desc, 32 * n); a.take(p.rightX, stereo ? n : 0); a.take(p.cellStart, kGridCells + 1); a.take(p.cellIdx, n);
  a.take(p.sortedKp, n); a.take(p.sortedDesc, 32 * n);
  a.take(p.queries, nq); a.take(p.qdesc, 32 * nq); a.take(p.taken, n + kTakenPad); a.take(p.assigned, n); a.take(p.matchQ, nq); a.take(p.qInfo, nq);
  a.take(p.qPre, nq); a.take(p.table, tableBytes); a.take(p.track, trackBytes);
  return a.L.bytes;
}

struct BowPtrs {
  int* status; CallDev* call;
  uint8_t *descA, *descB, *valid, *goodA, *goodB; KeyPointDev *kpsA, *kpsB; int *feat, *qFeat, *assigned, *matchQ; int2 *qRange, *qInfo; float* qAngle;
};
size_t layBow(size_t nA, size_t nB, size_t nFeatB, size_t nq, bool tri, void* base, BowPtrs& p) {
  Carve a(base);
  a.take(p.status, 16); a.take(p.call, 1);
  a.take(p.descA, 32 * nA); a.take(p.descB, 32 * nB); a.take(p.kpsB, nB); a.take(p.feat, nFeatB); a.take(p.valid, nB);
  a.take(p.qFeat, nq); a.take(p.qRange, nq); a.take(p.qAngle, nq); a.take(p.qInfo, nq); a.take(p.matchQ, nq); a.take(p.assigned, std::max(nq, nB));
  a.take(p.kpsA, tri ? nA : 0); a.take(p.goodA, tri ? nA : 0); a.take(p.goodB, tri ? nB : 0);
  return a.L.bytes;
}

struct RowsPtrs { uint8_t *a, *b; int *offsets, *idx, *out; TopkOut* top; };
size_t layRows(size_t nA, size_t nB, size_t nOffsets, size_t nIdx, size_t nOut, size_t nTop, void* base, RowsPtrs& r) {
  Carve a(base);
  a.take(r.a, 32 * nA); a.take(r.b, 32 * nB); a.take(r.offsets, nOffsets); a.take(r.idx, nIdx); a.take(r.out, nOut); a.take(r.top, nTop);
  return a.L.bytes;
}

struct StereoPtrs { int *counters, *kept, *status, *nL, *nR; KeyPointDev *kpsL, *kpsR; uint8_t *descL, *descR; float *rightX, *depth; };
size_t layStereo(size_t nPairs, size_t nl, size_t nr, void* base, StereoPtrs& p) {
  Carve a(base);
  a.take(p.counters, 4 * nPairs); a.take(p.kept, nPairs); a.take(p.status, nPairs);
  a.take(p.kpsL, nl); a.take(p.descL, 32 * nl); a.take(p.kpsR, nr); a.take(p.descR, 32 * nr); a.take(p.nL, nl ? nPairs : 0); a.take(p.nR, nl ? nPairs : 0);
  a.take(p.rightX, nl); a.take(p.depth, nl);
  return a.L.bytes;
}

}

struct ydorb_matcher {
  int device = 0;
  hipStream_t stream = nullptr;
  Mem call;
  Mem pool;
  size_t poolRecords = 1u << 20;
  Mem stereo;
  PinnedMem hUp, hDown;
  struct Batch {
    Mem arena;
    Mem status;
    std::vector<FrameDev> hFrames;
    std::vector<CallDev> hCalls;
    float hSf[8] = {0};
    bool hIdentAffine = false;
    BatchPtrs at{};
    int ovfPerKeypoint = 16;
  } batch;
  bool profiling = false;
  hipEvent_t ev[MS_COUNT + 1]{};
  double stageMs[MS_COUNT]{};
  int stageCalls = 0;
  bool evPending = false;
  std::vector<Mem*> buffers() { return {&call, &pool, &stereo, &hUp, &hDown, &batch.arena, &batch.status}; }
  ydorb_matcher() { for (Mem* b : buffers()) b->slackDiv = 2; }
};

static void collect(ydorb_matcher* m) {
  if (!m->profiling || !m->evPending) return;
  m->evPending = false;
  if (hipEventQuery(m->ev[MS_COUNT]) != hipSuccess) return;
  for (int i = 0; i < MS_COUNT; i++) {
    float ms = 0;
    if (hipEventElapsedTime(&ms, m->ev[i], m->ev[i + 1]) == hipSuccess) m->stageMs[i] += ms;
  }
  m->stageCalls++;
}

static bool validFrameView(const YdFrameView* fv) {
  return fv && fv->n >= 0 && (fv->n == 0 || (fv->kps && fv->desc)) && fv->max_x > fv->min_x && fv->max_y > fv->min_y;
}

extern "C" {

void ydorb_matcher_destroy(ydorb_matcher_t* m) {
  if (!m) return;
  (void)hipSetDevice(m->device);
  (void)hipStreamSynchronize(m->stream);
  for (Mem* b : m->buffers()) b->release();
  for (auto& e : m->ev) if (e) (void)hipEventDestroy(e);
  (void)hipStreamDestroy(m->stream);
  delete m;
}

int ydorb_matcher_create(int32_t device, ydorb_matcher_t** out) {
  if (!out) { set_error("null argument"); return YDORB_ERR_INVALID_ARG; }
  *out = nullptr;
  int rc = require_device(device);
  if (rc) return rc;
  ydorb_matcher* m = new ydorb_matcher();
  m->device = device;
  if (hipStreamCreateWithFlags(&m->stream, hipStreamNonBlocking) != hipSuccess) {
    set_error("hipStreamCreate failed");
    delete m;
    return YDORB_ERR_HIP;
  }
  for (auto& e : m->ev) (void)hipEventCreate(&e);
  if (m->batch.status.ensure(64) != YDORB_OK || hipMemset(m->batch.status.p, 0, 64) != hipSuccess) {
    set_error("matcher scratch allocation failed");
    ydorb_matcher_destroy(m);
    return YDORB_ERR_HIP;
  }
  *out = m;
  return YDORB_OK;
}

int ydorb_descriptor_distance(const uint8_t* a, const uint8_t* b) {
  int d = 0;
  for (int i = 0; i < 32; i += 8) {
    uint64_t x, y;
    memcpy(&x, a + i, 8);
    memcpy(&y, b + i, 8);
    d += __builtin_popcountll(x ^ y);
  }
  return d;
}

int ydorb_descriptor_distance_rows(ydorb_matcher_t* m, const uint8_t* a, const uint8_t* b, int32_t n, int32_t* out) {
  if (!m || !a || !b || !out || n < 0) { set_error("invalid argument"); return YDORB_ERR_INVALID_ARG; }
  if (n == 0) return YDORB_OK;
  HIPCHK(hipSetDevice(m->device));
  RowsPtrs r;
  if (const int rc = layOut(m->call, [&](void* base) { return layRows(n, n, 0, 0, n, 0, base, r); })) return rc;
  HIPCHK(hipMemcpyAsync(r.a, a, (size_t)32 * n, hipMemcpyHostToDevice, m->stream));
  HIPCHK(hipMemcpyAsync(r.b, b, (size_t)32 * n, hipMemcpyHostToDevice, m->stream));
  hipLaunchKernelGGL(k_hamming_rows, dim3((n + 255) / 256), dim3(256), 0, m->stream, r.a, r.b, n, r.out);
  HIPCHK(hipMemcpyAsync(out, r.out, sizeof(int) * n, hipMemcpyDeviceToHost, m->stream));
  HIPCHK(hipStreamSynchronize(m->stream));
  return YDORB_OK;
}

int ydorb_distinctive_descriptors(ydorb_matcher_t* m, const uint8_t* desc, const int32_t* offsets, int32_t nPoints, int32_t* best) {
  if (!m || !offsets || !best || nPoints < 0) { set_error("invalid argument"); return YDORB_ERR_INVALID_ARG; }
  if (nPoints == 0) return YDORB_OK;
  const int total = offsets[nPoints];
  if (offsets[0] != 0 || total < 0 || (total > 0 && !desc)) { set_error("invalid offsets"); return YDORB_ERR_INVALID_ARG; }
  for (int p = 0; p < nPoints; p++) {
    const int cnt = offsets[p + 1] - offsets[p];
    if (cnt < 0 || cnt > 65535) { set_error("map point %d holds %d descriptors (0..65535 supported)", p, cnt); return YDORB_ERR_INVALID_ARG; }
  }
  HIPCHK(hipSetDevice(m->device));
  RowsPtrs r;
  if (const int rc = layOut(m->call, [&](void* base) { return layRows(std::max(total, 1), 0, nPoints + 1, 0, nPoints, 0, base, r); })) return rc;
  if (total) HIPCHK(hipMemcpyAsync(r.a, desc, (size_t)32 * total, hipMemcpyHostToDevice, m->stream));
  HIPCHK(hipMemcpyAsync(r.offsets, offsets, sizeof(int) * (nPoints + 1), hipMemcpyHostToDevice, m->stream));
  hipLaunchKernelGGL(k_distinctive, dim3((nPoints + 3) / 4), dim3(256), 0, m->stream, r.a, r.offsets, nPoints, r.out);
  HIPCHK(hipGetLastError());
  HIPCHK(hipMemcpyAsync(best, r.out, sizeof(int) * nPoints, hipMemcpyDeviceToHost, m->stream));
  HIPCHK(hipStreamSynchronize(m->stream));
  return YDORB_OK;
}

static int searchProjectionImpl(ydorb_matcher_t* m, int32_t mode, const YdFrameView* fv, const YdQuery* queries, const uint8_t* qdesc,
                                int32_t nq, float ratio, int32_t orbDist, int32_t checkOri, uint8_t* taken, int32_t* assigned,
                                int32_t* nMatches, std::vector<uint32_t>* recordsOut, const float* invSigma2 = nullptr, int nLevels = 0,
                                int32_t* bestOut = nullptr, const ProjPtrs* laid = nullptr) {
  HIPCHK(hipSetDevice(m->device));
  const int n = fv->n;
  if (n > 65535) { set_error("frames with more than 65535 keypoints are not supported"); return YDORB_ERR_UNSUPPORTED; }
  if (nq == 0 || n == 0) { *nMatches = 0; return YDORB_OK; }
  int rc;
  ProjPtrs p;
  if (laid) p = *laid;
  else if ((rc = layOut(m->call, [&](void* base) { return layProjection(n, fv->right_x, nq, 0, 0, base, p); }))) return rc;
  for (int attempt = 0; attempt < 6; attempt++) {
    const size_t poolCap = (size_t)nq * kSlot + m->poolRecords;
    if ((rc = m->pool.ensure(sizeof(uint32_t) * poolCap))) return rc;
    HIPCHK(hipMemcpyAsync(p.kps, fv->kps, sizeof(YdKeyPoint) * n, hipMemcpyHostToDevice, m->stream));
    HIPCHK(hipMemcpyAsync(p.desc, fv->desc, (size_t)32 * n, hipMemcpyHostToDevice, m->stream));
    if (fv->right_x) HIPCHK(hipMemcpyAsync(p.rightX, fv->right_x, sizeof(float) * n, hipMemcpyHostToDevice, m->stream));
    FrameDev F{};
    F.kps = p.kps; F.desc = p.desc; F.rightX = fv->right_x ? p.rightX : nullptr; F.nPtr = nullptr; F.n = n;
    F.minX = fv->min_x; F.minY = fv->min_y;
    F.gridWInv = static_cast<float>(kGridCols) / (fv->max_x - fv->min_x);
    F.gridHInv = static_cast<float>(kGridRows) / (fv->max_y - fv->min_y);
    F.cellStart = p.cellStart; F.cellIdx = p.cellIdx; F.sortedKp = p.sortedKp; F.sortedDesc = p.sortedDesc;
    HIPCHK(hipMemcpyAsync(p.frame, &F, sizeof(FrameDev), hipMemcpyHostToDevice, m->stream));
    if ((rc = launchGridBuild(1, n, m->stream, p.frame))) return rc;
    HIPCHK(hipMemsetAsync(p.status, 0, 64, m->stream));
    if (queries) HIPCHK(hipMemcpyAsync(p.queries, queries, sizeof(YdQuery) * nq, hipMemcpyHostToDevice, m->stream));
    HIPCHK(hipMemcpyAsync(p.qdesc, qdesc, (size_t)32 * nq, hipMemcpyHostToDevice, m->stream));
    if (taken) HIPCHK(hipMemcpyAsync(p.taken, taken, n, hipMemcpyHostToDevice, m->stream));
    else HIPCHK(hipMemsetAsync(p.taken, 0, n, m->stream));
    if (assigned) HIPCHK(hipMemcpyAsync(p.assigned, assigned, sizeof(int) * n, hipMemcpyHostToDevice, m->stream));
    CallDev C{};
    C.tkps = p.kps; C.queries = p.queries; C.qdesc = p.qdesc; C.nq = nq; C.qInfo = p.qInfo; C.qPre = p.qPre;
    C.taken = p.taken; C.takenClear = taken ? 0 : 1; C.assigned = p.assigned; C.matchQ = p.matchQ;
    C.count = p.status + 2; C.mode = mode; C.ratio = ratio; C.orbDist = orbDist; C.checkOri = checkOri;
    for (int i = 0; i < 8; i++) C.invSigma2[i] = (invSigma2 && i < nLevels) ? invSigma2[i] : 0.f;
    HIPCHK(hipMemcpyAsync(p.call, &C, sizeof(CallDev), hipMemcpyHostToDevice, m->stream));
    hipLaunchKernelGGL(k_gather_projection, dim3((nq + 4 * kGatherQpw - 1) / (4 * kGatherQpw), 1), dim3(256), 0, m->stream, p.call, p.frame, nq,
                       m->pool.as<uint32_t>(), reinterpret_cast<unsigned*>(p.status), (unsigned)poolCap, p.status + 1);
    int hmisc[3];
    if (!recordsOut) {
      const int takenWords = (n + 31) / 32;
      hipLaunchKernelGGL(k_resolve, dim3(1), dim3(64), 2 * sizeof(unsigned) * takenWords, m->stream, p.call, p.frame, m->pool.as<uint32_t>(), takenWords);
    }
    HIPCHK(hipGetLastError());
    HIPCHK(hipMemcpyAsync(hmisc, p.status, sizeof(hmisc), hipMemcpyDeviceToHost, m->stream));
    HIPCHK(hipStreamSynchronize(m->stream));
    if (hmisc[1] != 0) {
      m->poolRecords = std::max<size_t>(m->poolRecords * 4, (size_t)(unsigned)hmisc[0] + 1024);
      continue;
    }
    if (recordsOut) {
      std::vector<int2> info(nq);
      HIPCHK(hipMemcpy(info.data(), p.qInfo, sizeof(int2) * nq, hipMemcpyDeviceToHost));
      recordsOut->resize(info[0].y);
      if (info[0].y) HIPCHK(hipMemcpy(recordsOut->data(), m->pool.as<uint32_t>() + info[0].x, sizeof(uint32_t) * info[0].y, hipMemcpyDeviceToHost));
      return YDORB_OK;
    }
    if (taken) HIPCHK(hipMemcpy(taken, p.taken, n, hipMemcpyDeviceToHost));
    if (assigned) HIPCHK(hipMemcpy(assigned, p.assigned, sizeof(int) * n, hipMemcpyDeviceToHost));
    if (bestOut) HIPCHK(hipMemcpy(bestOut, p.matchQ, sizeof(int) * nq, hipMemcpyDeviceToHost));
    *nMatches = hmisc[2];
    return YDORB_OK;
  }
  set_error("candidate record pool kept overflowing");
  return YDORB_ERR_CAPACITY;
}

struct BowJob {
  struct Side {
    const YdKeyPoint* kps; const uint8_t* desc; int n; const YdFeatureVector* fv;
    const uint8_t* ok;
    const uint8_t* good;
  } A, B;
  int mode;
  float ratio;
  int checkOri;
  BowCallDev geom;
};

static int bowSearch(ydorb_matcher_t* m, const BowJob& J, std::vector<int>& qFeat, std::vector<int>& res, int32_t* nMatches) {
  std::vector<int2> qRange;
  std::vector<float> qAngle;
  size_t records = 0;
  const YdFeatureVector &fa = *J.A.fv, &fb = *J.B.fv;
  for (int a = 0, b = 0; a < fa.n_nodes && b < fb.n_nodes;) {
    if (fa.node_ids[a] == fb.node_ids[b]) {
      for (int ia = fa.node_start[a]; ia < fa.node_start[a + 1]; ia++) {
        const int idxA = fa.feat[ia];
        if (!J.A.ok[idxA]) continue;
        qFeat.push_back(idxA);
        qRange.push_back(make_int2(fb.node_start[b], fb.node_start[b + 1]));
        qAngle.push_back(J.A.kps[idxA].angle);
        records += (size_t)(fb.node_start[b + 1] - fb.node_start[b]);
      }
      a++; b++;
    } else if (fa.node_ids[a] < fb.node_ids[b]) {
      a = (int)(std::lower_bound(fa.node_ids, fa.node_ids + fa.n_nodes, fb.node_ids[b]) - fa.node_ids);
    } else {
      b = (int)(std::lower_bound(fb.node_ids, fb.node_ids + fb.n_nodes, fa.node_ids[a]) - fb.node_ids);
    }
  }
  const int nq = (int)qFeat.size();
  if (nq == 0) return YDORB_OK;
  const int nFeatB = fb.node_start[fb.n_nodes], nA = J.A.n, nB = J.B.n;
  m->poolRecords = std::max<size_t>(m->poolRecords, records + 1024);
  int rc;
  BowPtrs p;
  if ((rc = layOut(m->call, [&](void* base) { return layBow(nA, nB, std::max(nFeatB, 1), nq, J.geom.tri, base, p); })) ||
      (rc = m->pool.ensure(sizeof(uint32_t) * m->poolRecords)))
    return rc;
  hipStream_t s = m->stream;
  HIPCHK(hipMemsetAsync(p.status, 0, 64, s));
  HIPCHK(hipMemcpyAsync(p.descA, J.A.desc, (size_t)32 * nA, hipMemcpyHostToDevice, s));
  HIPCHK(hipMemcpyAsync(p.descB, J.B.desc, (size_t)32 * nB, hipMemcpyHostToDevice, s));
  HIPCHK(hipMemcpyAsync(p.kpsB, J.B.kps, sizeof(YdKeyPoint) * nB, hipMemcpyHostToDevice, s));
  if (nFeatB) HIPCHK(hipMemcpyAsync(p.feat, fb.feat, sizeof(int) * nFeatB, hipMemcpyHostToDevice, s));
  if (J.B.ok) HIPCHK(hipMemcpyAsync(p.valid, J.B.ok, nB, hipMemcpyHostToDevice, s));
  HIPCHK(hipMemcpyAsync(p.qFeat, qFeat.data(), sizeof(int) * nq, hipMemcpyHostToDevice, s));
  HIPCHK(hipMemcpyAsync(p.qRange, qRange.data(), sizeof(int2) * nq, hipMemcpyHostToDevice, s));
  HIPCHK(hipMemcpyAsync(p.qAngle, qAngle.data(), sizeof(float) * nq, hipMemcpyHostToDevice, s));
  res.resize(std::max(nq, nB));
  HIPCHK(hipMemsetAsync(p.assigned, 0xFF, sizeof(int) * res.size(), s));
  BowCallDev BC = J.geom;
  BC.descA = p.descA; BC.descB = p.descB; BC.qFeat = p.qFeat; BC.qRange = p.qRange;
  BC.featB = p.feat; BC.validB = J.B.ok ? p.valid : nullptr; BC.nq = nq; BC.qInfo = p.qInfo;
  if (BC.tri) {
    HIPCHK(hipMemcpyAsync(p.kpsA, J.A.kps, sizeof(YdKeyPoint) * nA, hipMemcpyHostToDevice, s));
    HIPCHK(hipMemcpyAsync(p.goodA, J.A.good, nA, hipMemcpyHostToDevice, s));
    HIPCHK(hipMemcpyAsync(p.goodB, J.B.good, nB, hipMemcpyHostToDevice, s));
    BC.kpsA = p.kpsA; BC.kpsB = p.kpsB; BC.goodA = p.goodA; BC.goodB = p.goodB;
  }
  hipLaunchKernelGGL(k_gather_bow, dim3((nq + 3) / 4), dim3(256), 0, s, BC, m->pool.as<uint32_t>(), reinterpret_cast<unsigned*>(p.status),
                     (unsigned)m->poolRecords, p.status + 1);
  CallDev C{};
  C.tkps = p.kpsB; C.qAngle = p.qAngle; C.nq = nq; C.qInfo = p.qInfo; C.assigned = p.assigned; C.matchQ = p.matchQ;
  C.count = p.status + 2; C.mode = J.mode; C.ratio = J.ratio; C.checkOri = J.checkOri;
  HIPCHK(hipMemcpyAsync(p.call, &C, sizeof(CallDev), hipMemcpyHostToDevice, s));
  const int takenWords = (nB + 31) / 32;
  hipLaunchKernelGGL(k_resolve, dim3(1), dim3(64), 2 * sizeof(unsigned) * takenWords, s, p.call, (const FrameDev*)nullptr, m->pool.as<uint32_t>(), takenWords);
  HIPCHK(hipGetLastError());
  int hmisc[3];
  HIPCHK(hipMemcpyAsync(hmisc, p.status, sizeof(hmisc), hipMemcpyDeviceToHost, s));
  HIPCHK(hipMemcpyAsync(res.data(), p.assigned, sizeof(int) * res.size(), hipMemcpyDeviceToHost, s));
  HIPCHK(hipStreamSynchronize(s));
  if (hmisc[1] != 0) { set_error("bow record pool overflow"); return YDORB_ERR_CAPACITY; }
  *nMatches = hmisc[2];
  return YDORB_OK;
}

int ydorb_search_by_projection(ydorb_matcher_t* m, int32_t mode, const YdFrameView* fv, const YdQuery* queries, const uint8_t* qdesc,
                               int32_t nq, float ratio, int32_t orbDist, int32_t checkOri, uint8_t* taken, int32_t* assigned,
                               int32_t* nMatches) {
  if (!m || !validFrameView(fv) || !nMatches || mode < 0 || (mode > 2 && mode != 7) || nq < 0 || (nq > 0 && (!queries || !qdesc)) ||
      (fv->n > 0 && !assigned)) {
    set_error("invalid argument");
    return YDORB_ERR_INVALID_ARG;
  }
  if (mode == 7) checkOri = 0;
  return searchProjectionImpl(m, mode, fv, queries, qdesc, nq, ratio, orbDist, checkOri, taken, assigned, nMatches, nullptr);
}

int ydorb_search_local_points(ydorb_matcher_t* m, const YdFrameView* fv, const YdFrustumView* view, const YdMapPointTable* table,
                              const uint8_t* skip, const uint8_t* hasObs, float th, float ratio, uint8_t* taken, int32_t* assigned,
                              YdTrackView* rows, uint8_t* status, int32_t* nToMatch, int32_t* nMatches) {
  if (!m || !fv || !view || !table || !nToMatch || !nMatches) { set_error("search_local_points: null argument"); return YDORB_ERR_INVALID_ARG; }
  if (view->n_levels < 1 || view->n_levels > 8) { set_error("search_local_points: n_levels %d outside 1..8", view->n_levels); return YDORB_ERR_INVALID_ARG; }
  const int np = table->n, n = fv->n;
  if (np < 0 || n < 0) { set_error("search_local_points: negative size"); return YDORB_ERR_INVALID_ARG; }
  if (np > 0 && (!table->pos_min || !table->normal_max || !table->max_distance || !table->desc || !skip || !hasObs || !rows || !status)) {
    set_error("search_local_points: null map-point table, flag or output arrays");
    return YDORB_ERR_INVALID_ARG;
  }
  if (!validFrameView(fv) || (n > 0 && !assigned)) {
    set_error("search_local_points: invalid frame view");
    return YDORB_ERR_INVALID_ARG;
  }
  *nToMatch = 0; *nMatches = 0;
  if (np == 0) return YDORB_OK;
  HIPCHK(hipSetDevice(m->device));
  const size_t p = np;
  Layout U;
  const size_t oPos = U.add(16 * p), oNrm = U.add(16 * p), oMax = U.add(4 * p), oSkip = U.add(p), oObs = U.add(p);
  Layout D;
  const size_t dRows = D.add(sizeof(YdTrackView) * p), dSt = D.add(p);
  int rc;
  ProjPtrs q;
  if ((rc = m->hUp.ensure(U.bytes)) || (rc = m->hDown.ensure(D.bytes))) return rc;
  if ((rc = layOut(m->call, [&](void* base) { return layProjection(std::max(n, 1), fv->right_x, np, U.bytes, D.bytes, base, q); }))) return rc;
  std::memcpy(at<void>(m->hUp, oPos), table->pos_min, 16 * p);
  std::memcpy(at<void>(m->hUp, oNrm), table->normal_max, 16 * p);
  std::memcpy(at<void>(m->hUp, oMax), table->max_distance, 4 * p);
  std::memcpy(at<void>(m->hUp, oSkip), skip, p);
  std::memcpy(at<void>(m->hUp, oObs), hasObs, p);
  HIPCHK(hipMemcpyAsync(q.table, m->hUp.p, U.bytes, hipMemcpyHostToDevice, m->stream));
  hipLaunchKernelGGL(frustum::k_frustum_queries<QueryDev>, dim3((np + frustum::kThreads - 1) / frustum::kThreads), dim3(frustum::kThreads), 0, m->stream, *view,
                     np, (const float4*)(q.table + oPos), (const float4*)(q.table + oNrm), (const float*)(q.table + oMax), q.table + oSkip, q.table + oObs, th,
                     q.queries, (YdTrackView*)(q.track + dRows), q.track + dSt);
  HIPCHK(hipGetLastError());
  HIPCHK(hipMemcpyAsync(m->hDown.p, q.track, D.bytes, hipMemcpyDeviceToHost, m->stream));
  if ((rc = searchProjectionImpl(m, YDORB_SEARCH_FRAME_MAPPOINT, fv, nullptr, table->desc, np, ratio, 0, 0, taken, assigned, nMatches, nullptr, nullptr, 0,
                                 nullptr, &q)))
    return rc;
  HIPCHK(hipStreamSynchronize(m->stream));
  std::memcpy(rows, at<void>(m->hDown, dRows), sizeof(YdTrackView) * p);
  std::memcpy(status, at<void>(m->hDown, dSt), p);
  for (int i = 0; i < np; i++) *nToMatch += status[i] == YDORB_FRUSTUM_IN_VIEW;
  return YDORB_OK;
}

int ydorb_fuse_search(ydorb_matcher_t* m, const YdFrameView* fv, const YdQuery* queries, const uint8_t* qdesc, int32_t nq,
                      const float* invSigma2, int32_t nLevels, int32_t* best, int32_t* nFound) {
  return ydorb_window_search(m, fv, queries, qdesc, nq, invSigma2, nLevels, 50, best, nFound);
}

int ydorb_window_search(ydorb_matcher_t* m, const YdFrameView* fv, const YdQuery* queries, const uint8_t* qdesc, int32_t nq,
                        const float* invSigma2, int32_t nLevels, int32_t maxDist, int32_t* best, int32_t* nFound) {
  if (!m || !validFrameView(fv) || !nFound || nq < 0 || maxDist < 0 || maxDist > 256 || (nq > 0 && (!queries || !qdesc || !best)) || !invSigma2 || nLevels < 1 ||
      nLevels > 8) {
    set_error("invalid argument");
    return YDORB_ERR_INVALID_ARG;
  }
  for (int q = 0; q < nq; q++) best[q] = -1;
  *nFound = 0;
  for (int i = 0; i < fv->n; i++)
    if (fv->kps[i].octave < 0 || fv->kps[i].octave >= nLevels) { set_error("keyframe feature %d: octave %d outside the %d-level table", i, fv->kps[i].octave, nLevels); return YDORB_ERR_INVALID_ARG; }
  return searchProjectionImpl(m, 6, fv, queries, qdesc, nq, 0.f, maxDist, 0, nullptr, nullptr, nFound, nullptr, invSigma2, nLevels, best);
}

int ydorb_frame_keypoints_in_area(ydorb_matcher_t* m, const YdFrameView* fv, float x, float y, float r, int32_t minLevel, int32_t maxLevel,
                                  int32_t* outIdx, int32_t cap, int32_t* nOut) {
  if (!m || !validFrameView(fv) || !nOut || (cap > 0 && !outIdx)) {
    set_error("invalid argument");
    return YDORB_ERR_INVALID_ARG;
  }
  *nOut = 0;
  if (fv->n == 0) return YDORB_OK;
  YdQuery q{};
  q.u = x; q.v = y; q.r = r; q.min_level = minLevel; q.max_level = maxLevel; q.flags = 1;
  uint8_t zero[32] = {0};
  std::vector<uint32_t> rec;
  int dummy = 0;
  int rc = searchProjectionImpl(m, 2, fv, &q, zero, 1, 0.f, 0, 0, nullptr, nullptr, &dummy, &rec);
  if (rc) return rc;
  if ((int)rec.size() > cap) { set_error("%zu candidates, capacity %d", rec.size(), cap); return YDORB_ERR_CAPACITY; }
  for (size_t i = 0; i < rec.size(); i++) outIdx[i] = (int)(rec[i] & 0xFFFFu);
  *nOut = (int)rec.size();
  return YDORB_OK;
}

int ydorb_search_by_bow(ydorb_matcher_t* m, int32_t mode, const YdBowSide* A, const YdBowSide* B, float ratio, int32_t checkOri, int32_t* out,
                        int32_t* nMatches) {
  if (!m || !A || !B || !out || !nMatches || (mode != 3 && mode != 4) || A->n < 0 || B->n < 0 || (A->n > 0 && (!A->kps || !A->desc || !A->valid)) ||
      (B->n > 0 && (!B->kps || !B->desc)) || (mode == 4 && B->n > 0 && !B->valid)) {
    set_error("invalid argument");
    return YDORB_ERR_INVALID_ARG;
  }
  HIPCHK(hipSetDevice(m->device));
  const int nOutLen = mode == 3 ? B->n : A->n;
  for (int i = 0; i < nOutLen; i++) out[i] = -1;
  *nMatches = 0;
  if (A->n == 0 || B->n == 0) return YDORB_OK;
  if (B->n > 65535) { set_error("more than 65535 features per frame are not supported"); return YDORB_ERR_UNSUPPORTED; }
  const BowJob J{{A->kps, A->desc, A->n, &A->fv, A->valid, nullptr}, {B->kps, B->desc, B->n, &B->fv, mode == 4 ? B->valid : nullptr, nullptr}, mode, ratio, checkOri, {}};
  std::vector<int> qFeat, res;
  const int rc = bowSearch(m, J, qFeat, res, nMatches);
  if (rc || qFeat.empty()) return rc;
  if (mode == 3) {
    for (int i = 0; i < B->n; i++) out[i] = res[i] >= 0 ? qFeat[res[i]] : -1;
  } else {
    for (size_t q = 0; q < qFeat.size(); q++) out[qFeat[q]] = res[q];
  }
  return YDORB_OK;
}

int ydorb_search_for_triangulation(ydorb_matcher_t* m, const YdTriSide* A, const YdTriSide* B, const float* F, float ex, float ey,
                                   const float* sfB, const float* sf2B, int32_t nLevels, int32_t stereoOnly, int32_t checkOri, int32_t* out,
                                   int32_t* nMatches) {
  if (!m || !A || !B || !F || !sfB || !sf2B || !out || !nMatches || nLevels < 1 || nLevels > 8 || A->n < 0 || B->n < 0 ||
      (A->n > 0 && (!A->kps || !A->desc || !A->right_x || !A->has_map_point)) || (B->n > 0 && (!B->kps || !B->desc || !B->right_x || !B->has_map_point))) {
    set_error("invalid argument");
    return YDORB_ERR_INVALID_ARG;
  }
  HIPCHK(hipSetDevice(m->device));
  for (int i = 0; i < A->n; i++) out[i] = -1;
  *nMatches = 0;
  if (A->n == 0 || B->n == 0) return YDORB_OK;
  if (B->n > 65535) { set_error("more than 65535 features per frame are not supported"); return YDORB_ERR_UNSUPPORTED; }
  for (int i = 0; i < B->n; i++)
    if (B->kps[i].octave < 0 || B->kps[i].octave >= nLevels) { set_error("second keyframe: octave %d outside the %d-level tables", B->kps[i].octave, nLevels); return YDORB_ERR_INVALID_ARG; }
  std::vector<uint8_t> goodA(A->n), goodB(B->n), eligibleA(A->n), validB(B->n);
  for (int i = 0; i < A->n; i++) { goodA[i] = A->right_x[i] >= 0; eligibleA[i] = !A->has_map_point[i] && (!stereoOnly || goodA[i]); }
  for (int i = 0; i < B->n; i++) { goodB[i] = B->right_x[i] >= 0; validB[i] = !B->has_map_point[i] && (!stereoOnly || goodB[i]); }
  BowJob J{{A->kps, A->desc, A->n, &A->fv, eligibleA.data(), goodA.data()}, {B->kps, B->desc, B->n, &B->fv, validB.data(), goodB.data()}, 5, 0.f, checkOri, {}};
  J.geom.tri = 1;
  for (int i = 0; i < 9; i++) J.geom.F[i] = F[i];
  J.geom.ex = ex; J.geom.ey = ey;
  for (int i = 0; i < 8; i++) { J.geom.sfB[i] = i < nLevels ? sfB[i] : 0.f; J.geom.sf2B[i] = i < nLevels ? sf2B[i] : 0.f; }
  std::vector<int> qFeat, res;
  const int rc = bowSearch(m, J, qFeat, res, nMatches);
  if (rc) return rc;
  for (size_t q = 0; q < qFeat.size(); q++) out[qFeat[q]] = res[q];
  return YDORB_OK;
}

int ydorb_stereo_matches(ydorb_matcher_t* m, const YdStereoSide* L, const YdStereoSide* R, int32_t nPairs, float bf, float b, int32_t flags,
                         float* rightX, float* depth, int32_t* nKept, int32_t* status, void* stream) {
  if (!m || !L || !R || !L->extractor || !R->extractor || !L->kps || !L->desc || !L->n || !R->kps || !R->desc || !R->n || !rightX || !depth ||
      nPairs < 1 || L->cap < 1 || R->cap < 1 || !(bf > 0.f) || !(b > 0.f)) {
    set_error("invalid argument");
    return YDORB_ERR_INVALID_ARG;
  }
  if (R->cap > kStereoMaxRight) { set_error("right cap %d > %d", R->cap, kStereoMaxRight); return YDORB_ERR_CAPACITY; }
  PyramidView vl, vr;
  int rc;
  if ((rc = extractor_pyramid_view(L->extractor, &vl)) || (rc = extractor_pyramid_view(R->extractor, &vr))) return rc;
  if (vl.device != m->device || vr.device != m->device) { set_error("extractors and matcher live on different devices"); return YDORB_ERR_INVALID_ARG; }
  if (vl.nLevels != vr.nLevels) { set_error("left and right pyramids differ in depth"); return YDORB_ERR_INVALID_ARG; }
  for (int l = 0; l < vl.nLevels; l++)
    if (vl.w[l] != vr.w[l] || vl.h[l] != vr.h[l] || vl.scale[l] != vr.scale[l]) { set_error("left and right pyramids differ at level %d", l); return YDORB_ERR_INVALID_ARG; }
  const int lastL = L->first_frame + (nPairs - 1) * L->frame_step, lastR = R->first_frame + (nPairs - 1) * R->frame_step;
  if (L->first_frame < 0 || lastL < 0 || L->first_frame >= vl.frames || lastL >= vl.frames || R->first_frame < 0 || lastR < 0 ||
      R->first_frame >= vr.frames || lastR >= vr.frames) {
    set_error("pair frames outside the extractors' last call (%d / %d frames)", vl.frames, vr.frames);
    return YDORB_ERR_INVALID_ARG;
  }
  HIPCHK(hipSetDevice(m->device));
  const bool dev = flags & YDORB_STEREO_DEVICE_POINTERS;
  hipStream_t s = stream ? (hipStream_t)stream : m->stream;
  const size_t nl = (size_t)nPairs * L->cap, nr = (size_t)nPairs * R->cap;
  StereoPtrs sp;
  if ((rc = layOut(m->stereo, [&](void* base) { return layStereo(nPairs, dev ? 0 : nl, dev ? 0 : nr, base, sp); }))) return rc;
  StereoDev P{};
  if (dev) {
    P.kpsL = reinterpret_cast<const KeyPointDev*>(L->kps); P.descL = L->desc; P.nL = L->n;
    P.kpsR = reinterpret_cast<const KeyPointDev*>(R->kps); P.descR = R->desc; P.nR = R->n;
    P.rightX = rightX; P.depth = depth;
  } else {
    HIPCHK(hipStreamSynchronize((hipStream_t)vl.stream));
    HIPCHK(hipStreamSynchronize((hipStream_t)vr.stream));
    HIPCHK(hipMemcpyAsync(sp.kpsL, L->kps, sizeof(YdKeyPoint) * nl, hipMemcpyHostToDevice, s));
    HIPCHK(hipMemcpyAsync(sp.descL, L->desc, 32 * nl, hipMemcpyHostToDevice, s));
    HIPCHK(hipMemcpyAsync(sp.kpsR, R->kps, sizeof(YdKeyPoint) * nr, hipMemcpyHostToDevice, s));
    HIPCHK(hipMemcpyAsync(sp.descR, R->desc, 32 * nr, hipMemcpyHostToDevice, s));
    HIPCHK(hipMemcpyAsync(sp.nL, L->n, sizeof(int) * nPairs, hipMemcpyHostToDevice, s));
    HIPCHK(hipMemcpyAsync(sp.nR, R->n, sizeof(int) * nPairs, hipMemcpyHostToDevice, s));
    P.kpsL = sp.kpsL; P.descL = sp.descL; P.nL = sp.nL;
    P.kpsR = sp.kpsR; P.descR = sp.descR; P.nR = sp.nR;
    P.rightX = sp.rightX; P.depth = sp.depth;
  }
  for (int l = 0; l < vl.nLevels; l++) {
    P.pyrL[l] = vl.roi[l]; P.pyrR[l] = vr.roi[l];
    P.w[l] = vl.w[l]; P.h[l] = vl.h[l]; P.pitchL[l] = vl.pitch[l]; P.pitchR[l] = vr.pitch[l];
    P.scale[l] = vl.scale[l]; P.invScale[l] = vl.invScale[l];
  }
  P.frameStrideL = vl.frameStride; P.frameStrideR = vr.frameStride;
  P.capL = L->cap; P.capR = R->cap; P.frameL0 = L->first_frame; P.frameLStep = L->frame_step; P.frameR0 = R->first_frame; P.frameRStep = R->frame_step;
  P.nLevels = vl.nLevels; P.flags = flags; P.bf = bf; P.maxD = bf / b;
  P.counters = sp.counters; P.keptOut = sp.kept; P.statusOut = sp.status;
  size_t ldsReplay = (size_t)R->cap * 8;
  {
    const size_t bytes = (size_t)R->cap * 8 + sizeof(int) * (2 * (size_t)vl.h[0] + 1) + 2 * (size_t)R->cap + 16;
    const bool noLists = getenv("YDORB_STEREO_NO_ROW_LISTS") != nullptr;
    if (!noLists && !(flags & YDORB_STEREO_INDEX_BY_KEYPOINT) && bytes <= 120 * 1024 && vl.h[0] < 4095) { P.rowLists = 1; ldsReplay = bytes; }
  }
  HIPCHK(hipMemsetAsync(sp.counters, 0, sizeof(int) * 4 * nPairs, s));
  HIPCHK(hipMemsetD32Async(reinterpret_cast<hipDeviceptr_t>(P.rightX), 0xBF800000u, nl, s));
  HIPCHK(hipMemsetD32Async(reinterpret_cast<hipDeviceptr_t>(P.depth), 0xBF800000u, nl, s));
  const size_t lds = (size_t)R->cap * 8;
  const StereoDev& dP = P;
  if (lds > 48 * 1024) HIPCHK(hipFuncSetAttribute(reinterpret_cast<const void*>(&k_stereo<false>), hipFuncAttributeMaxDynamicSharedMemorySize, (int)lds));
  if (ldsReplay > 48 * 1024) HIPCHK(hipFuncSetAttribute(reinterpret_cast<const void*>(&k_stereo<true>), hipFuncAttributeMaxDynamicSharedMemorySize, (int)ldsReplay));
  if (flags & YDORB_STEREO_INDEX_BY_KEYPOINT)
    hipLaunchKernelGGL(k_stereo<false>, dim3((L->cap + kStereoChunk - 1) / kStereoChunk, nPairs), dim3(256), lds, s, dP, 0, 0);
  else {
    const char* sliceStr = getenv("YDORB_STEREO_SLICE");
    const int sliceEnv = sliceStr ? atoi(sliceStr) : 0;
    const int slice = sliceEnv > 0 ? sliceEnv : (nPairs >= 8 ? 1024 : L->cap);
    for (int k0 = 0; k0 < L->cap; k0 += slice)
      hipLaunchKernelGGL(k_stereo<true>, dim3(1, nPairs), dim3(256), ldsReplay, s, dP, k0, std::min(k0 + slice, L->cap));
  }
  hipLaunchKernelGGL(k_stereo_outliers, dim3(nPairs), dim3(256), 0, s, P);
  HIPCHK(hipGetLastError());
  if (dev) {
    if (nKept) HIPCHK(hipMemcpyAsync(nKept, P.keptOut, sizeof(int) * nPairs, hipMemcpyDeviceToDevice, s));
    if (status) HIPCHK(hipMemcpyAsync(status, P.statusOut, sizeof(int) * nPairs, hipMemcpyDeviceToDevice, s));
    return YDORB_OK;
  }
  HIPCHK(hipMemcpyAsync(rightX, P.rightX, sizeof(float) * nl, hipMemcpyDeviceToHost, s));
  HIPCHK(hipMemcpyAsync(depth, P.depth, sizeof(float) * nl, hipMemcpyDeviceToHost, s));
  if (nKept) HIPCHK(hipMemcpyAsync(nKept, P.keptOut, sizeof(int) * nPairs, hipMemcpyDeviceToHost, s));
  if (status) HIPCHK(hipMemcpyAsync(status, P.statusOut, sizeof(int) * nPairs, hipMemcpyDeviceToHost, s));
  HIPCHK(hipStreamSynchronize(s));
  return YDORB_OK;
}

int ydorb_match_pairs_device(ydorb_matcher_t* m, const YdFrameSetDev* Q, const YdFrameSetDev* T, const int32_t* pairs, int32_t nCalls,
                             int32_t width, int32_t height, float th, const float* scaleFactors, int32_t nLevels, const float* d_affine,
                             int32_t checkOri, int32_t* d_assigned, int32_t* d_counts, void* stream) {
  if (!m || !Q || !T || !pairs || !Q->d_kps || !Q->d_desc || !Q->d_n || !T->d_kps || !T->d_desc || !T->d_n || !d_assigned || !d_counts || !scaleFactors ||
      Q->cap < 1 || Q->cap > 65535 || T->cap != Q->cap || Q->n_frames < 1 || T->n_frames < 1 || nCalls < 1 || nLevels < 1 || nLevels > 8 || width < 1 ||
      height < 1) {
    set_error("invalid argument");
    return YDORB_ERR_INVALID_ARG;
  }
  for (int c = 0; c < nCalls; c++)
    if (pairs[2 * c] < 0 || pairs[2 * c] >= Q->n_frames || pairs[2 * c + 1] < 0 || pairs[2 * c + 1] >= T->n_frames) {
      set_error("pair %d references a frame out of range", c);
      return YDORB_ERR_INVALID_ARG;
    }
  HIPCHK(hipSetDevice(m->device));
  hipStream_t s = stream ? (hipStream_t)stream : m->stream;
  std::vector<int> tmap(T->n_frames, -1);
  std::vector<int> tused;
  for (int c = 0; c < nCalls; c++) {
    const int tf = pairs[2 * c + 1];
    if (tmap[tf] < 0) { tmap[tf] = (int)tused.size(); tused.push_back(tf); }
  }
  auto& B = m->batch;
  const int cap = Q->cap, nFrames = (int)tused.size();
  const size_t poolPerCall = (size_t)cap * kSlot + (size_t)cap * B.ovfPerKeypoint;
  BatchPtrs p;
  const size_t had = B.arena.cap;
  const int rc = layOut(B.arena, [&](void* base) { return layBatch(cap, nCalls, nFrames, poolPerCall, base, p); });
  if (B.arena.cap != had) B.hFrames.clear();
  if (rc) return rc;
  std::vector<FrameDev> hf(nFrames);
  std::vector<CallDev> hc(nCalls);
  const float minX = 0.f, minY = 0.f, maxX = (float)width, maxY = (float)height;
  for (int f = 0; f < nFrames; f++) {
    const int tf = tused[f];
    FrameDev& F = hf[f];
    F.kps = reinterpret_cast<const KeyPointDev*>(T->d_kps) + (size_t)tf * cap; F.desc = T->d_desc + (size_t)tf * cap * 32; F.rightX = nullptr;
    F.nPtr = T->d_n + tf; F.n = 0; F.minX = minX; F.minY = minY;
    F.gridWInv = static_cast<float>(kGridCols) / (maxX - minX); F.gridHInv = static_cast<float>(kGridRows) / (maxY - minY);
    F.cellStart = p.cellStart + (size_t)f * (kGridCells + 1); F.cellIdx = p.cellIdx + (size_t)f * cap;
    F.sortedKp = p.sortedKp + (size_t)f * cap; F.sortedDesc = p.sortedDesc + (size_t)f * cap * 32;
  }
  for (int c = 0; c < nCalls; c++) {
    const int qf = pairs[2 * c], tf = tmap[pairs[2 * c + 1]];
    CallDev& C = hc[c];
    C.frame = tf; C.tkps = hf[tf].kps; C.qAngle = nullptr; C.queries = p.queries + (size_t)c * cap;
    C.qkps = reinterpret_cast<const KeyPointDev*>(Q->d_kps) + (size_t)qf * cap;
    C.qdesc = Q->d_desc + (size_t)qf * cap * 32; C.nqPtr = Q->d_n + qf; C.nq = 0; C.qInfo = p.qInfo + (size_t)c * cap;
    C.qPre = p.qPre + (size_t)c * cap; C.takenClear = 1;
    C.taken = p.taken + (size_t)c * cap; C.assigned = d_assigned + (size_t)c * cap; C.matchQ = p.matchQ + (size_t)c * cap;
    C.count = d_counts + c; C.mode = 1; C.ratio = 0.9f; C.orbDist = 0; C.checkOri = checkOri;
  }
// ... 142 lines not shown
```

Before: 182.6.

## Coalesce host-device transfers into single pinned staging copies and inline quadtree for small batches

The matcher's many small per-array uploads and downloads are replaced by packing inputs into a pinned host twin of the device arena. The arena is then moved with one H2D copy and one D2H copy, with buffers reordered so the in and out regions are contiguous. The extractor merges its nOut, keypoint and descriptor readback into one copy and folds the passList memset into the describe kernel. It also defaults to inline quadtree streams for small batches, dropping event records. This cuts per-call API and DMA launch overhead, at the cost of extra host memcpy into staging and transferring some padding bytes.

```diff
diff --git a/ydorbslam_amd/csrc/extract_kernels.hip.h b/ydorbslam_amd/csrc/extract_kernels.hip.h
--- a/ydorbslam_amd/csrc/extract_kernels.hip.h
+++ b/ydorbslam_amd/csrc/extract_kernels.hip.h
@@ -1280,7 +1280,7 @@
                                                          const uint8_t* __restrict__ blur, size_t blurFrameStride, PlanDev P,
                                                          const uint32_t* __restrict__ lvlKp, const int* __restrict__ lvlCount,
                                                          YdKeyPointDev* __restrict__ kps, uint8_t* __restrict__ desc, int cap,
-                                                         int* __restrict__ nOut, float* __restrict__ lvlAngle) {
+                                                         int* __restrict__ nOut, float* __restrict__ lvlAngle, int* __restrict__ passCount) {
   const int lane = threadIdx.x & 63;
   int bx = blockIdx.x, f = blockIdx.y;
   if ((f | 7) < (int)gridDim.y) {
@@ -1305,7 +1305,10 @@
     if (l == level) mine = c;
     tot += c;
   }
-  if (slot == 0 && lane == 0) nOut[f] = min(tot, cap);
+  if (slot == 0 && lane == 0) {
+    nOut[f] = min(tot, cap);
+    if (passCount && f == 0) *passCount = 0;
+  }
   const LevelDev L = P.lv[level];
   const int k = slot - L.kpOff;
   if (k >= mine) return;
@@ -1380,7 +1383,7 @@
                                                            const uint8_t* __restrict__ blur, size_t blurFrameStride, PlanDev P,
                                                            const uint32_t* __restrict__ lvlKp, const int* __restrict__ lvlCount,
                                                            YdKeyPointDev* __restrict__ kps, uint8_t* __restrict__ desc, int cap,
-                                                           int* __restrict__ nOut, float* __restrict__ lvlAngle) {
+                                                           int* __restrict__ nOut, float* __restrict__ lvlAngle, int* __restrict__ passCount) {
   const int lane = threadIdx.x & 63;
   int bx = blockIdx.x, f = blockIdx.y;
   if ((f | 7) < (int)gridDim.y) {
@@ -1407,7 +1410,10 @@
       if (l < P.nLevels && slot >= P.lv[l].kpOff) level[j] = l;
     pk[j] = __builtin_amdgcn_readfirstlane(lvlKp[(size_t)f * P.sumQuota + slot]);
   }
-  if (slot0 == 0 && lane == 0) nOut[f] = min(tot, cap);
+  if (slot0 == 0 && lane == 0) {
+    nOut[f] = min(tot, cap);
+    if (passCount && f == 0) *passCount = 0;
+  }
   bool any = false;
 #pragma unroll
   for (int j = 0; j < KPW; j++) {
diff --git a/ydorbslam_amd/csrc/orb_extractor.hip b/ydorbslam_amd/csrc/orb_extractor.hip
--- a/ydorbslam_amd/csrc/orb_extractor.hip
+++ b/ydorbslam_amd/csrc/orb_extractor.hip
@@ -65,15 +65,18 @@
   a.take(w.cellCount, D.nCellsTotal * B); a.take(w.cellCand, (size_t)D.nCellsTotal * D.cellCap * B);
   a.take(w.qtCand, 2 * P.qtFrameStride * B); a.take(w.qtNode, 2 * P.qtFrameStride * B); a.take(w.nodeScratch, D.nodeTabFrameStride * B);
   a.take(w.lvlKp, D.sumQuota * B); a.take(w.lvlAngle, D.sumQuota * B); a.take(w.lvlCount, kMaxLevels * B);
-  a.take(w.needPass, kMaxLevels * B); a.take(w.lvlMaxN, kMaxLevels + 1); a.take(w.status, 1); a.take(w.passList, kMaxLevels * B + 1);
+  a.take(w.needPass, kMaxLevels * B); a.take(w.lvlMaxN, kMaxLevels + 2); w.status = w.lvlMaxN + kMaxLevels + 1; a.take(w.passList, kMaxLevels * B + 1);
   return a.L.bytes;
 }
 
-struct IoPtrs { uint8_t* img; YdKeyPoint* kps; uint8_t* desc; int* nOut; };
-size_t layIo(size_t imgBytes, size_t Q, size_t B, void* base, IoPtrs& p) {
+struct IoPtrs { uint8_t* img; int* nOut; YdKeyPoint* kps; uint8_t* desc; size_t outBytes; };
+size_t layIo(size_t imgBytes, size_t Q, size_t B, size_t n, void* base, IoPtrs& p) {
   static_assert(sizeof(YdKeyPoint) == sizeof(YdKeyPointDev), "one layout for the device and the pinned staging");
   Carve a(base);
-  a.take(p.img, imgBytes * B); a.take(p.kps, Q * B); a.take(p.desc, 32 * Q * B); a.take(p.nOut, B);
+  a.take(p.img, imgBytes * B);
+  const size_t out0 = a.L.bytes;
+  a.take(p.nOut, n); a.take(p.kps, Q * n); a.take(p.desc, 32 * Q * n);
+  p.outBytes = a.L.bytes - out0;
   return a.L.bytes;
 }
 
@@ -415,13 +418,14 @@
   return YDORB_OK;
 }
 
-int ensureIo(ydorb_extractor* e) {
-  if (e->io.p && e->hIo.p) return YDORB_OK;
-  const size_t bytes = layIo(e->imgBytes, e->sumQuota, e->batchCap, nullptr, e->dIo);
-  int rc;
-  if ((rc = e->io.alloc(bytes)) || (rc = e->hIo.alloc(bytes))) return rc;
-  layIo(e->imgBytes, e->sumQuota, e->batchCap, e->io.p, e->dIo);
-  layIo(e->imgBytes, e->sumQuota, e->batchCap, e->hIo.p, e->hIoAt);
+int ensureIo(ydorb_extractor* e, int nFrames) {
+  if (!e->io.p || !e->hIo.p) {
+    const size_t bytes = layIo(e->imgBytes, e->sumQuota, e->batchCap, e->batchCap, nullptr, e->dIo);
+    int rc;
+    if ((rc = e->io.alloc(bytes)) || (rc = e->hIo.alloc(bytes))) return rc;
+  }
+  layIo(e->imgBytes, e->sumQuota, e->batchCap, nFrames, e->io.p, e->dIo);
+  layIo(e->imgBytes, e->sumQuota, e->batchCap, nFrames, e->hIo.p, e->hIoAt);
   return YDORB_OK;
 }
 
@@ -490,7 +494,7 @@
         if (narrow) hipLaunchKernelGGL(k_fast_cells<48>, grid, dim3(256), dyn, s, e->d.pyr, P.pyrFrameStride, D, e->tab.cells, c0, c1, thr, fl, e->d.cellCount, e->d.cellCand);
         else hipLaunchKernelGGL(k_fast_cells<80>, grid, dim3(256), dyn, s, e->d.pyr, P.pyrFrameStride, D, e->tab.cells, c0, c1, thr, fl, e->d.cellCount, e->d.cellCand);
       }
-      HIPCHK(hipEventRecord(e->evFast[l0], s));
+      if (!e->qtInline) HIPCHK(hipEventRecord(e->evFast[l0], s));
       fastEv[l0] = e->evFast[l0];
       grpFirst[nGroups] = l0; grpEnd[nGroups] = l1; nGroups++;
       for (int l = l0 + 1; l < l1; l++) fastEv[l] = e->evFast[l0];
@@ -498,7 +502,7 @@
     }
   }
   if (prof) HIPCHK(hipEventRecord(e->ev[2], s));
-  HIPCHK(hipEventRecord(e->evFork, s));
+  if (!e->qtInline) HIPCHK(hipEventRecord(e->evFork, s));
   hipLaunchKernelGGL(k_blur, dim3((D.blurTileBegin[D.nLevels] + 7) / 8 * 8, nFrames), dim3(256), 0, s, e->d.pyr, P.pyrFrameStride, e->d.blur,
                      P.blurFrameStride, D);
   if (prof) HIPCHK(hipEventRecord(e->ev[3], s));
@@ -538,23 +542,23 @@
     hipLaunchKernelGGL(k_quadtree_list, dim3(listGrid), dim3(kQtListThreads), P.qtPassLds, s, D, e->d.cellCount, e->d.cellCand,
                        e->d.qtCand, e->d.qtNode, P.qtFrameStride, -std::max(P.qtPassNodes, 1), e->d.lvlKp, e->d.lvlCount, e->d.status, e->d.passList,
                        e->d.passList + 1, e->d.nodeScratch, e->d.lvlMaxN + kMaxLevels);
-    HIPCHK(hipMemsetAsync(e->d.passList, 0, sizeof(int), s));
   }
   if (prof) HIPCHK(hipEventRecord(e->ev[4], s));
   {
     const int kpw = e->descKpw;
     const dim3 gd(((D.sumQuota + 4 * kpw - 1) / (4 * kpw) + 7) / 8 * 8, nFrames);
+    int* const passCount = anyFast ? e->d.passList : nullptr;
 #define YD_DESC(K) hipLaunchKernelGGL((k_orient_describe_n<K>), gd, dim3(256), 0, s, e->d.pyr, P.pyrFrameStride, e->d.blur, P.blurFrameStride, D, \
-                                         e->d.lvlKp, e->d.lvlCount, d_kps, d_desc, cap, d_nOut, e->d.lvlAngle)
+                                         e->d.lvlKp, e->d.lvlCount, d_kps, d_desc, cap, d_nOut, e->d.lvlAngle, passCount)
     if (kpw == 1)
       hipLaunchKernelGGL(k_orient_describe, gd, dim3(256), 0, s, e->d.pyr, P.pyrFrameStride, e->d.blur,
-                         P.blurFrameStride, D, e->d.lvlKp, e->d.lvlCount, d_kps, d_desc, cap, d_nOut, e->d.lvlAngle);
+                         P.blurFrameStride, D, e->d.lvlKp, e->d.lvlCount, d_kps, d_desc, cap, d_nOut, e->d.lvlAngle, passCount);
     else if (kpw == 2) YD_DESC(2);
     else YD_DESC(4);
 #undef YD_DESC
   }
   if (prof) { HIPCHK(hipEventRecord(e->ev[5], s)); e->profPending = true; }
-  HIPCHK(hipMemcpyAsync(e->h_lvlMaxN, e->d.lvlMaxN, sizeof(int) * (kMaxLevels + 1), hipMemcpyDeviceToHost, s));
+  HIPCHK(hipMemcpyAsync(e->h_lvlMaxN, e->d.lvlMaxN, sizeof(int) * (kMaxLevels + 2), hipMemcpyDeviceToHost, s));
   HIPCHK(hipGetLastError());
   e->lastFrames = nFrames;
   e->lastStream = s;
@@ -652,8 +656,8 @@
   (void)hipEventCreateWithFlags(&e->evFork, hipEventDisableTiming);
   for (int l = 0; l < kMaxLevels; l++) {
     const char* qtEnv = getenv("YDORB_QT_STREAMS");
-    e->qtInline = (qtEnv && atoi(qtEnv) == 0) || (cfg->flags & YDORB_EXTRACTOR_SINGLE_STREAM);
-    const int nQt = std::max(1, std::min(qtEnv ? atoi(qtEnv) : (cfg->max_batch <= 8 ? (int)kMaxLevels : 2), (int)kMaxLevels));
+    e->qtInline = (qtEnv ? atoi(qtEnv) == 0 : cfg->max_batch <= 8) || (cfg->flags & YDORB_EXTRACTOR_SINGLE_STREAM);
+    const int nQt = std::max(1, std::min(qtEnv ? atoi(qtEnv) : 2, (int)kMaxLevels));
     if (l < nQt) (void)hipStreamCreateWithFlags(&e->qtStream[l], hipStreamNonBlocking);
     else e->qtStream[l] = e->qtStream[l % nQt];
     (void)hipEventCreateWithFlags(&e->evJoin[l], hipEventDisableTiming);
@@ -737,7 +741,7 @@
   if (!kps || !desc || stride < w) { set_error("invalid argument"); return YDORB_ERR_INVALID_ARG; }
   HIPCHK(hipSetDevice(e->cfg.device));
   int rc = ensurePlan(e, w, h, n_frames);
-  if (rc || (rc = ensureIo(e))) return rc;
+  if (rc || (rc = ensureIo(e, n_frames))) return rc;
   const int Q = e->sumQuota;
   YdKeyPointDev* d_kps = reinterpret_cast<YdKeyPointDev*>(e->dIo.kps);
   for (int f = 0; f < n_frames; f++)
@@ -745,10 +749,7 @@
   HIPCHK(hipMemcpyAsync(e->dIo.img, e->hIoAt.img, e->imgBytes * n_frames, hipMemcpyHostToDevice, e->stream));
   rc = enqueue(e, e->dIo.img, w, e->imgBytes, n_frames, d_kps, e->dIo.desc, Q, e->dIo.nOut, e->stream);
   if (rc) return rc;
-  HIPCHK(hipMemcpyAsync(e->hIoAt.nOut, e->dIo.nOut, sizeof(int) * n_frames, hipMemcpyDeviceToHost, e->stream));
-  HIPCHK(hipMemcpyAsync(e->h_status, e->d.status, sizeof(int), hipMemcpyDeviceToHost, e->stream));
-  HIPCHK(hipMemcpyAsync(e->hIoAt.kps, d_kps, sizeof(YdKeyPoint) * (size_t)Q * n_frames, hipMemcpyDeviceToHost, e->stream));
-  HIPCHK(hipMemcpyAsync(e->hIoAt.desc, e->dIo.desc, (size_t)32 * Q * n_frames, hipMemcpyDeviceToHost, e->stream));
+  HIPCHK(hipMemcpyAsync(e->hIoAt.nOut, e->dIo.nOut, e->dIo.outBytes, hipMemcpyDeviceToHost, e->stream));
   HIPCHK(hipStreamSynchronize(e->stream));
   collectProfile(e);
   rc = checkStatus(e);
diff --git a/ydorbslam_amd/csrc/orb_matcher.hip b/ydorbslam_amd/csrc/orb_matcher.hip
--- a/ydorbslam_amd/csrc/orb_matcher.hip
+++ b/ydorbslam_amd/csrc/orb_matcher.hip
@@ -59,33 +59,43 @@
 }
 
 struct ProjPtrs {
-  int* status; FrameDev* frame; CallDev* call;
-  KeyPointDev* kps; uint8_t* desc; float* rightX; int *cellStart, *cellIdx; float4* sortedKp; uint8_t* sortedDesc;
-  QueryDev* queries; uint8_t *qdesc, *taken; int *assigned, *matchQ; int2* qInfo; uint2* qPre;
+  QueryDev* queries; FrameDev* frame; CallDev* call;
+  KeyPointDev* kps; uint8_t* desc; float* rightX; uint8_t* qdesc;
+  int* status; uint8_t* taken; int *assigned, *matchQ;
+  int *cellStart, *cellIdx; float4* sortedKp; uint8_t* sortedDesc; int2* qInfo; uint2* qPre;
   uint8_t *table, *track;
 };
 size_t layProjection(size_t n, bool stereo, size_t nq, size_t tableBytes, size_t trackBytes, void* base, ProjPtrs& p) {
   Carve a(base);
-  a.take(p.status, 16); a.take(p.frame, 1); a.take(p.call, 1);
-  a.take(p.kps, n); a.take(p.desc, 32 * n); a.take(p.rightX, stereo ? n : 0); a.take(p.cellStart, kGridCells + 1); a.take(p.cellIdx, n);
-  a.take(p.sortedKp, n); a.take(p.sortedDesc, 32 * n);
-  a.take(p.queries, nq); a.take(p.qdesc, 32 * nq); a.take(p.taken, n + kTakenPad); a.take(p.assigned, n); a.take(p.matchQ, nq); a.take(p.qInfo, nq);
+  a.take(p.queries, nq); a.take(p.frame, 1); a.take(p.call, 1);
+  a.take(p.kps, n); a.take(p.desc, 32 * n); a.take(p.rightX, stereo ? n : 0); a.take(p.qdesc, 32 * nq);
+  a.take(p.status, 16); a.take(p.taken, n + kTakenPad); a.take(p.assigned, n); a.take(p.matchQ, nq);
+  a.take(p.cellStart, kGridCells + 1); a.take(p.cellIdx, n); a.take(p.sortedKp, n); a.take(p.sortedDesc, 32 * n); a.take(p.qInfo, nq);
   a.take(p.qPre, nq); a.take(p.table, tableBytes); a.take(p.track, trackBytes);
   return a.L.bytes;
 }
 
 struct BowPtrs {
-  int* status; CallDev* call;
-  uint8_t *descA, *descB, *valid, *goodA, *goodB; KeyPointDev *kpsA, *kpsB; int *feat, *qFeat, *assigned, *matchQ; int2 *qRange, *qInfo; float* qAngle;
+  CallDev* call;
+  uint8_t *descA, *descB, *valid, *goodA, *goodB; KeyPointDev *kpsA, *kpsB; int *feat, *qFeat; int2* qRange; float* qAngle;
+  int *status, *assigned, *matchQ; int2* qInfo;
 };
 size_t layBow(size_t nA, size_t nB, size_t nFeatB, size_t nq, bool tri, void* base, BowPtrs& p) {
   Carve a(base);
-  a.take(p.status, 16); a.take(p.call, 1);
+  a.take(p.call, 1);
   a.take(p.descA, 32 * nA); a.take(p.descB, 32 * nB); a.take(p.kpsB, nB); a.take(p.feat, nFeatB); a.take(p.valid, nB);
-  a.take(p.qFeat, nq); a.take(p.qRange, nq); a.take(p.qAngle, nq); a.take(p.qInfo, nq); a.take(p.matchQ, nq); a.take(p.assigned, std::max(nq, nB));
+  a.take(p.qFeat, nq); a.take(p.qRange, nq); a.take(p.qAngle, nq);
   a.take(p.kpsA, tri ? nA : 0); a.take(p.goodA, tri ? nA : 0); a.take(p.goodB, tri ? nB : 0);
+  a.take(p.status, 16); a.take(p.assigned, std::max(nq, nB));
+  a.take(p.matchQ, nq); a.take(p.qInfo, nq);
   return a.L.bytes;
 }
+
+struct Twin {
+  uint8_t *dev, *host;
+  size_t off(const void* d) const { return (size_t)(static_cast<const uint8_t*>(d) - dev); }
+  template <class T> T* operator()(T* d) const { return reinterpret_cast<T*>(host + off(d)); }
+};
 
 struct RowsPtrs { uint8_t *a, *b; int *offsets, *idx, *out; TopkOut* top; };
 size_t layRows(size_t nA, size_t nB, size_t nOffsets, size_t nIdx, size_t nOut, size_t nTop, void* base, RowsPtrs& r) {
@@ -113,6 +123,7 @@
   size_t poolRecords = 1u << 20;
   Mem stereo;
   PinnedMem hUp, hDown;
+  PinnedMem hCallUp, hCallDown;
   struct Batch {
     Mem arena;
     Mem status;
@@ -128,7 +139,7 @@
   double stageMs[MS_COUNT]{};
   int stageCalls = 0;
   bool evPending = false;
-  std::vector<Mem*> buffers() { return {&call, &pool, &stereo, &hUp, &hDown, &batch.arena, &batch.status}; }
+  std::vector<Mem*> buffers() { return {&call, &pool, &stereo, &hUp, &hDown, &hCallUp, &hCallDown, &batch.arena, &batch.status}; }
   ydorb_matcher() { for (Mem* b : buffers()) b->slackDiv = 2; }
 };
 
@@ -239,42 +250,55 @@
   ProjPtrs p;
   if (laid) p = *laid;
   else if ((rc = layOut(m->call, [&](void* base) { return layProjection(n, fv->right_x, nq, 0, 0, base, p); }))) return rc;
-  for (int attempt = 0; attempt < 6; attempt++) {
-    const size_t poolCap = (size_t)nq * kSlot + m->poolRecords;
-    if ((rc = m->pool.ensure(sizeof(uint32_t) * poolCap))) return rc;
-    HIPCHK(hipMemcpyAsync(p.kps, fv->kps, sizeof(YdKeyPoint) * n, hipMemcpyHostToDevice, m->stream));
-    HIPCHK(hipMemcpyAsync(p.desc, fv->desc, (size_t)32 * n, hipMemcpyHostToDevice, m->stream));
-    if (fv->right_x) HIPCHK(hipMemcpyAsync(p.rightX, fv->right_x, sizeof(float) * n, hipMemcpyHostToDevice, m->stream));
+  const bool stereo = fv->right_x != nullptr;
+  Twin tw{m->call.as<uint8_t>(), nullptr};
+  const size_t oUp = tw.off(queries ? (const void*)p.queries : (const void*)p.frame), oRedo = tw.off(p.status);
+  const size_t oUpEnd = assigned ? tw.off(p.assigned) + sizeof(int) * n : tw.off(p.taken) + n + kTakenPad;
+  const size_t downBytes = recordsOut ? 64 : tw.off(p.matchQ) + sizeof(int) * nq - oRedo;
+  if ((rc = m->hCallUp.ensure(oUpEnd)) || (rc = m->hCallDown.ensure(downBytes))) return rc;
+  tw.host = m->hCallUp.as<uint8_t>();
+  const uint8_t* const down = m->hCallDown.as<uint8_t>();
+  {
     FrameDev F{};
-    F.kps = p.kps; F.desc = p.desc; F.rightX = fv->right_x ? p.rightX : nullptr; F.nPtr = nullptr; F.n = n;
+    F.kps = p.kps; F.desc = p.desc; F.rightX = stereo ? p.rightX : nullptr; F.nPtr = nullptr; F.n = n;
     F.minX = fv->min_x; F.minY = fv->min_y;
     F.gridWInv = static_cast<float>(kGridCols) / (fv->max_x - fv->min_x);
     F.gridHInv = static_cast<float>(kGridRows) / (fv->max_y - fv->min_y);
     F.cellStart = p.cellStart; F.cellIdx = p.cellIdx; F.sortedKp = p.sortedKp; F.sortedDesc = p.sortedDesc;
-    HIPCHK(hipMemcpyAsync(p.frame, &F, sizeof(FrameDev), hipMemcpyHostToDevice, m->stream));
-    if ((rc = launchGridBuild(1, n, m->stream, p.frame))) return rc;
-    HIPCHK(hipMemsetAsync(p.status, 0, 64, m->stream));
-    if (queries) HIPCHK(hipMemcpyAsync(p.queries, queries, sizeof(YdQuery) * nq, hipMemcpyHostToDevice, m->stream));
-    HIPCHK(hipMemcpyAsync(p.qdesc, qdesc, (size_t)32 * nq, hipMemcpyHostToDevice, m->stream));
-    if (taken) HIPCHK(hipMemcpyAsync(p.taken, taken, n, hipMemcpyHostToDevice, m->stream));
-    else HIPCHK(hipMemsetAsync(p.taken, 0, n, m->stream));
-    if (assigned) HIPCHK(hipMemcpyAsync(p.assigned, assigned, sizeof(int) * n, hipMemcpyHostToDevice, m->stream));
     CallDev C{};
     C.tkps = p.kps; C.queries = p.queries; C.qdesc = p.qdesc; C.nq = nq; C.qInfo = p.qInfo; C.qPre = p.qPre;
     C.taken = p.taken; C.takenClear = taken ? 0 : 1; C.assigned = p.assigned; C.matchQ = p.matchQ;
     C.count = p.status + 2; C.mode = mode; C.ratio = ratio; C.orbDist = orbDist; C.checkOri = checkOri;
     for (int i = 0; i < 8; i++) C.invSigma2[i] = (invSigma2 && i < nLevels) ? invSigma2[i] : 0.f;
-    HIPCHK(hipMemcpyAsync(p.call, &C, sizeof(CallDev), hipMemcpyHostToDevice, m->stream));
+    if (queries) std::memcpy(tw(p.queries), queries, sizeof(YdQuery) * nq);
+    std::memcpy(tw(p.frame), &F, sizeof(FrameDev));
+    std::memcpy(tw(p.call), &C, sizeof(CallDev));
+    std::memcpy(tw(p.kps), fv->kps, sizeof(YdKeyPoint) * n);
+    std::memcpy(tw(p.desc), fv->desc, (size_t)32 * n);
+    if (stereo) std::memcpy(tw(p.rightX), fv->right_x, sizeof(float) * n);
+    std::memcpy(tw(p.qdesc), qdesc, (size_t)32 * nq);
+    std::memset(tw(p.status), 0, 64);
+    if (taken) std::memcpy(tw(p.taken), taken, n);
+    else std::memset(tw(p.taken), 0, n);
+    std::memset(tw(p.taken) + n, 0, kTakenPad);
+    if (assigned) std::memcpy(tw(p.assigned), assigned, sizeof(int) * n);
+  }
+  for (int attempt = 0; attempt < 6; attempt++) {
+    const size_t poolCap = (size_t)nq * kSlot + m->poolRecords;
+    if ((rc = m->pool.ensure(sizeof(uint32_t) * poolCap))) return rc;
+    const size_t from = attempt == 0 ? oUp : oRedo;
+    HIPCHK(hipMemcpyAsync(tw.dev + from, tw.host + from, oUpEnd - from, hipMemcpyHostToDevice, m->stream));
+    if (attempt == 0 && (rc = launchGridBuild(1, n, m->stream, p.frame))) return rc;
     hipLaunchKernelGGL(k_gather_projection, dim3((nq + 4 * kGatherQpw - 1) / (4 * kGatherQpw), 1), dim3(256), 0, m->stream, p.call, p.frame, nq,
                        m->pool.as<uint32_t>(), reinterpret_cast<unsigned*>(p.status), (unsigned)poolCap, p.status + 1);
-    int hmisc[3];
     if (!recordsOut) {
       const int takenWords = (n + 31) / 32;
       hipLaunchKernelGGL(k_resolve, dim3(1), dim3(64), 2 * sizeof(unsigned) * takenWords, m->stream, p.call, p.frame, m->pool.as<uint32_t>(), takenWords);
     }
     HIPCHK(hipGetLastError());
-    HIPCHK(hipMemcpyAsync(hmisc, p.status, sizeof(hmisc), hipMemcpyDeviceToHost, m->stream));
+    HIPCHK(hipMemcpyAsync(m->hCallDown.p, p.status, downBytes, hipMemcpyDeviceToHost, m->stream));
     HIPCHK(hipStreamSynchronize(m->stream));
+    const int* hmisc = reinterpret_cast<const int*>(down);
     if (hmisc[1] != 0) {
       m->poolRecords = std::max<size_t>(m->poolRecords * 4, (size_t)(unsigned)hmisc[0] + 1024);
       continue;
@@ -286,9 +310,9 @@
       if (info[0].y) HIPCHK(hipMemcpy(recordsOut->data(), m->pool.as<uint32_t>() + info[0].x, sizeof(uint32_t) * info[0].y, hipMemcpyDeviceToHost));
       return YDORB_OK;
     }
-    if (taken) HIPCHK(hipMemcpy(taken, p.taken, n, hipMemcpyDeviceToHost));
-    if (assigned) HIPCHK(hipMemcpy(assigned, p.assigned, sizeof(int) * n, hipMemcpyDeviceToHost));
-    if (bestOut) HIPCHK(hipMemcpy(bestOut, p.matchQ, sizeof(int) * nq, hipMemcpyDeviceToHost));
+    if (taken) std::memcpy(taken, down + (tw.off(p.taken) - oRedo), n);
+    if (assigned) std::memcpy(assigned, down + (tw.off(p.assigned) - oRedo), sizeof(int) * n);
+    if (bestOut) std::memcpy(bestOut, down + (tw.off(p.matchQ) - oRedo), sizeof(int) * nq);
     *nMatches = hmisc[2];
     return YDORB_OK;
   }
@@ -340,39 +364,44 @@
       (rc = m->pool.ensure(sizeof(uint32_t) * m->poolRecords)))
     return rc;
   hipStream_t s = m->stream;
-  HIPCHK(hipMemsetAsync(p.status, 0, 64, s));
-  HIPCHK(hipMemcpyAsync(p.descA, J.A.desc, (size_t)32 * nA, hipMemcpyHostToDevice, s));
-  HIPCHK(hipMemcpyAsync(p.descB, J.B.desc, (size_t)32 * nB, hipMemcpyHostToDevice, s));
-  HIPCHK(hipMemcpyAsync(p.kpsB, J.B.kps, sizeof(YdKeyPoint) * nB, hipMemcpyHostToDevice, s));
-  if (nFeatB) HIPCHK(hipMemcpyAsync(p.feat, fb.feat, sizeof(int) * nFeatB, hipMemcpyHostToDevice, s));
-  if (J.B.ok) HIPCHK(hipMemcpyAsync(p.valid, J.B.ok, nB, hipMemcpyHostToDevice, s));
-  HIPCHK(hipMemcpyAsync(p.qFeat, qFeat.data(), sizeof(int) * nq, hipMemcpyHostToDevice, s));
-  HIPCHK(hipMemcpyAsync(p.qRange, qRange.data(), sizeof(int2) * nq, hipMemcpyHostToDevice, s));
-  HIPCHK(hipMemcpyAsync(p.qAngle, qAngle.data(), sizeof(float) * nq, hipMemcpyHostToDevice, s));
   res.resize(std::max(nq, nB));
-  HIPCHK(hipMemsetAsync(p.assigned, 0xFF, sizeof(int) * res.size(), s));
+  Twin tw{m->call.as<uint8_t>(), nullptr};
+  const size_t oDown = tw.off(p.status), oUpEnd = tw.off(p.assigned) + sizeof(int) * res.size();
+  if ((rc = m->hCallUp.ensure(oUpEnd)) || (rc = m->hCallDown.ensure(oUpEnd - oDown))) return rc;
+  tw.host = m->hCallUp.as<uint8_t>();
   BowCallDev BC = J.geom;
   BC.descA = p.descA; BC.descB = p.descB; BC.qFeat = p.qFeat; BC.qRange = p.qRange;
   BC.featB = p.feat; BC.validB = J.B.ok ? p.valid : nullptr; BC.nq = nq; BC.qInfo = p.qInfo;
-  if (BC.tri) {
-    HIPCHK(hipMemcpyAsync(p.kpsA, J.A.kps, sizeof(YdKeyPoint) * nA, hipMemcpyHostToDevice, s));
-    HIPCHK(hipMemcpyAsync(p.goodA, J.A.good, nA, hipMemcpyHostToDevice, s));
-    HIPCHK(hipMemcpyAsync(p.goodB, J.B.good, nB, hipMemcpyHostToDevice, s));
-    BC.kpsA = p.kpsA; BC.kpsB = p.kpsB; BC.goodA = p.goodA; BC.goodB = p.goodB;
-  }
-  hipLaunchKernelGGL(k_gather_bow, dim3((nq + 3) / 4), dim3(256), 0, s, BC, m->pool.as<uint32_t>(), reinterpret_cast<unsigned*>(p.status),
-                     (unsigned)m->poolRecords, p.status + 1);
   CallDev C{};
   C.tkps = p.kpsB; C.qAngle = p.qAngle; C.nq = nq; C.qInfo = p.qInfo; C.assigned = p.assigned; C.matchQ = p.matchQ;
   C.count = p.status + 2; C.mode = J.mode; C.ratio = J.ratio; C.checkOri = J.checkOri;
-  HIPCHK(hipMemcpyAsync(p.call, &C, sizeof(CallDev), hipMemcpyHostToDevice, s));
+  std::memcpy(tw(p.call), &C, sizeof(CallDev));
+  std::memcpy(tw(p.descA), J.A.desc, (size_t)32 * nA);
+  std::memcpy(tw(p.descB), J.B.desc, (size_t)32 * nB);
+  std::memcpy(tw(p.kpsB), J.B.kps, sizeof(YdKeyPoint) * nB);
+  if (nFeatB) std::memcpy(tw(p.feat), fb.feat, sizeof(int) * nFeatB);
+  if (J.B.ok) std::memcpy(tw(p.valid), J.B.ok, nB);
+  std::memcpy(tw(p.qFeat), qFeat.data(), sizeof(int) * nq);
+  std::memcpy(tw(p.qRange), qRange.data(), sizeof(int2) * nq);
+  std::memcpy(tw(p.qAngle), qAngle.data(), sizeof(float) * nq);
+  if (BC.tri) {
+    std::memcpy(tw(p.kpsA), J.A.kps, sizeof(YdKeyPoint) * nA);
+    std::memcpy(tw(p.goodA), J.A.good, nA);
+    std::memcpy(tw(p.goodB), J.B.good, nB);
+    BC.kpsA = p.kpsA; BC.kpsB = p.kpsB; BC.goodA = p.goodA; BC.goodB = p.goodB;
+  }
+  std::memset(tw(p.status), 0, 64);
+  std::memset(tw(p.assigned), 0xFF, sizeof(int) * res.size());
+  HIPCHK(hipMemcpyAsync(tw.dev, tw.host, oUpEnd, hipMemcpyHostToDevice, s));
+  hipLaunchKernelGGL(k_gather_bow, dim3((nq + 3) / 4), dim3(256), 0, s, BC, m->pool.as<uint32_t>(), reinterpret_cast<unsigned*>(p.status),
+                     (unsigned)m->poolRecords, p.status + 1);
   const int takenWords = (nB + 31) / 32;
   hipLaunchKernelGGL(k_resolve, dim3(1), dim3(64), 2 * sizeof(unsigned) * takenWords, s, p.call, (const FrameDev*)nullptr, m->pool.as<uint32_t>(), takenWords);
   HIPCHK(hipGetLastError());
-  int hmisc[3];
-  HIPCHK(hipMemcpyAsync(hmisc, p.status, sizeof(hmisc), hipMemcpyDeviceToHost, s));
-  HIPCHK(hipMemcpyAsync(res.data(), p.assigned, sizeof(int) * res.size(), hipMemcpyDeviceToHost, s));
+  HIPCHK(hipMemcpyAsync(m->hCallDown.p, p.status, oUpEnd - oDown, hipMemcpyDeviceToHost, s));
   HIPCHK(hipStreamSynchronize(s));
+  const int* hmisc = m->hCallDown.as<int>();
+  std::memcpy(res.data(), m->hCallDown.as<uint8_t>() + (tw.off(p.assigned) - oDown), sizeof(int) * res.size());
   if (hmisc[1] != 0) { set_error("bow record pool overflow"); return YDORB_ERR_CAPACITY; }
   *nMatches = hmisc[2];
   return YDORB_OK;
```

Result: no change. 182.5 (median of 2 runs) (-0.0%).
